# facebookresearch/iSDF

Measured on AMD Instinct MI355X. Metric: train-steps/sec: device-synchronised Trainer.step() on 27k-point ray batches, timed as metrics.start_timing / end_timing bracket it (SURVEY 8d); whole job.  SDF L1 vs GT: sdf_l1_vs_gt, higher is better.
Workload: dtype f16 MFMA operands (compensated forward: hi+lo operands past the cat layer), f32 accumulate; second-order sweeps and dW operands fp16; 1 GPU; replicaCAD.json defaults: 5 keyframes x 200 rays x 27 samples = 27000 points per rank-step, 680x1200 synthetic room depth, 6x256 Softplus MLP + 255-wide icosahedron PE (460033 params), eik+normal loss, bounds=ray, AdamW; stream=680x1200, scaling_mode=weak: every rank draws the full 5 x 200 rays, parallelism=single GPU

## Files before the change

### include/isdf_hip.h

```cpp
#ifndef ISDF_HIP_H
#define ISDF_HIP_H

#include <stddef.h>
#include <stdint.h>

#ifdef __cplusplus
extern "C" {
#endif

#define ISDF_ABI_VERSION 7

enum {
  ISDF_OK = 0,
  ISDF_EINVAL = -1,
  ISDF_EUNSUPPORTED = -2,
  ISDF_EWORKSPACE = -3,
  ISDF_EHIP = -4,
  ISDF_ECOLLECTIVE = -5
};

typedef struct isdf_net_cfg {
  int32_t hidden;
  int32_t blocks;
  int32_t n_freqs;
  int32_t has_transform;
  float scale_input;
  float scale_output;
  float bounds_T[12];
  int32_t fwd_operand;
  int32_t bwd_operand;
  int32_t spill_operand;
} isdf_net_cfg;

int isdf_abi_version(void);
const char* isdf_error_string(int code);

int isdf_check_net(const isdf_net_cfg* net);

int64_t isdf_param_count(const isdf_net_cfg* net);
int64_t isdf_shadow_bytes(const isdf_net_cfg* net);
int64_t isdf_workspace_bytes(const isdf_net_cfg* net, int64_t max_points, int32_t train);
int64_t isdf_reduce_floats(const isdf_net_cfg* net, int32_t n_frames);
int64_t isdf_reduce_split_floats(const isdf_net_cfg* net);

int isdf_pack_weights(const isdf_net_cfg* net, const float* params, void* shadow, void* stream);

typedef struct isdf_sample_args {
  const float* depth_batch;
  const float* normal_batch;
  const float* T_WC_batch;
  const int32_t* frame_idx;
  const int32_t* normal_idx;
  int32_t n_frames;
  int32_t n_rays;
  int32_t H, W;
  float fx, fy, cx, cy;
  int32_t n_strat, n_surf;
  float min_depth;
  float dist_behind_surf;
  int32_t rng_mode;
  const int64_t* draw_h;
  const int64_t* draw_w;
  const float* draw_u;
  const float* draw_n;
  uint64_t seed, offset;
  int32_t n_inline;
  int32_t frame_idx_inline[8];
  int32_t normal_idx_inline[8];
  int32_t reserved_inline;
} isdf_sample_args;
#define ISDF_MAX_INLINE_FRAMES 8

typedef struct isdf_sample_out {
  int32_t* n_valid;
  int64_t* indices_b;
  int64_t* indices_h;
  int64_t* indices_w;
  float* depth_sample;
  float* dirs_C_sample;
  float* norm_sample;
  float* T_WC_sample;
  float* dirs_W_sample;
  float* z_vals;
  float* pc;
} isdf_sample_out;

int64_t isdf_sample_scan_bytes(int64_t max_rays);
int isdf_sample_rays(const isdf_sample_args* a, const isdf_sample_out* o, void* scan_ws,
                     int64_t scan_ws_bytes, void* stream);

int isdf_sdf_eval(const isdf_net_cfg* net, const float* params, const void* shadow,
                  const float* pts, int64_t n_points, const float* noise,
                  float* sdf, float* sdf_grad, void* workspace, int64_t workspace_bytes,
                  void* stream);

typedef struct isdf_loss_cfg {
  int32_t bounds_method;
  int32_t loss_type;
  float trunc_weight, trunc_distance, eik_weight, eik_apply_dist, grad_weight;
  int32_t orien_loss;
} isdf_loss_cfg;

typedef struct isdf_step_args {
  const int32_t* n_valid;
  int32_t max_rays;
  int32_t S;
  int32_t n_frames, H, W;
  const float* pc;
  const float* z_vals;
  const float* depth_sample;
  const float* dirs_C_sample;
  const float* dirs_W_sample;
  const float* norm_sample;
  const int64_t* indices_b;
  const int64_t* indices_h;
  const int64_t* indices_w;
  const float* noise;
  float noise_std;
  uint32_t reserved0;
  uint64_t noise_seed;
  uint64_t noise_offset;
  const float* pc_bounds;
  const float* pc_grad_vec;
  int32_t extra_floats;
  int32_t extra_slot;
  float extra_value;
  int32_t reserved1;
} isdf_step_args;

typedef struct isdf_step_out {
  float* reduce_buf;
  float* sdf;
  float* sdf_grad;
  float* tot_loss_mat;
  void** prof_events;
  float* host_mailbox;
  void* split_event;
} isdf_step_out;

enum { ISDF_LS_SDF = 0, ISDF_LS_GRAD = 1, ISDF_LS_EIK = 2, ISDF_LS_TOTAL = 3, ISDF_LS_COUNT = 4 };

int isdf_train_step(const isdf_net_cfg* net, const isdf_loss_cfg* loss, const float* params,
                    const void* shadow, const isdf_step_args* a, const isdf_step_out* o,
                    void* workspace, int64_t workspace_bytes, void* stream);

typedef struct isdf_optim_args {
  float* params;
  float* exp_avg;
  float* exp_avg_sq;
  void* shadow;
  float lr, beta1, beta2, eps, weight_decay;
  float grad_scale;
  int32_t step;
  int32_t reserved;
  float* loss_approx;
  float* frame_avg;
  const int32_t* frame_avg_index;
  int32_t frame_avg_inline_n;
  int32_t frame_avg_index_inline[8];
  int32_t reserved_inline;
} isdf_optim_args;

int isdf_train_step_adamw(const isdf_net_cfg* net, const isdf_loss_cfg* loss, const isdf_step_args* a,
                          const isdf_step_out* o, const isdf_optim_args* opt, void* workspace,
                          int64_t workspace_bytes, void* stream);

int isdf_train_step_finish(const isdf_net_cfg* net, const isdf_optim_args* opt, const float* reduce_buf,
                           int32_t n_frames, int32_t extra_floats, float* host_mailbox, void* stream);

typedef int (*isdf_nccl_allreduce_fn)(const void* sendbuf, void* recvbuf, size_t count, int datatype, int op,
                                      void* comm, void* stream);
int isdf_allreduce_sum_f32(isdf_nccl_allreduce_fn nccl_all_reduce, void* comm, float* buf, int64_t count, void* stream);

int isdf_bounds_pc(const int32_t* n_valid, int32_t max_rays, int32_t S, const float* pc,
                   const float* z_vals, const float* depth_sample, const float* surf_pts,
                   int64_t n_surf, float* bounds, float* grad_vec, void* stream);

int isdf_frame_avg(const float* reduce_buf, int64_t n_params, int32_t n_frames,
                   float* loss_approx, float* frame_avg_loss, const int32_t* frame_avg_index,
                   void* stream);

int isdf_estimate_normals(const float* depth, int32_t H, int32_t W, float fx, float fy, float cx,
                          float cy, float* normals, void* stream);

int isdf_render_depth(const int32_t* n_valid, int64_t n_rays_host, int64_t max_rays, int32_t S,
                      const float* z_vals, const float* sdf, const float* depth_sample,
                      float kf_dist_th, float* view_depth, int32_t* below_count, void* stream);

int isdf_adamw(const isdf_net_cfg* net, float* params, float* exp_avg, float* exp_avg_sq,
               const float* grad_sum, const float* count_ptr, float grad_scale,
               float lr, float beta1, float beta2, float eps, float weight_decay,
               int32_t step, void* shadow, void* stream);

#ifdef __cplusplus
}
#endif
#endif
```

### isdf_amd/_ffi.py

```python
import ctypes as C
import os

HERE = os.path.dirname(os.path.abspath(__file__))
LIB_PATH = os.environ.get("ISDF_HIP_LIB") or os.path.join(HERE, "libisdf_hip.so")

ABI_VERSION = 7

SYMBOLS = [
    "isdf_abi_version", "isdf_error_string", "isdf_check_net", "isdf_param_count", "isdf_shadow_bytes",
    "isdf_workspace_bytes", "isdf_reduce_floats", "isdf_reduce_split_floats", "isdf_sample_scan_bytes", "isdf_pack_weights",
    "isdf_sample_rays",
    "isdf_sdf_eval", "isdf_train_step", "isdf_train_step_adamw", "isdf_train_step_finish", "isdf_bounds_pc",
    "isdf_frame_avg", "isdf_adamw", "isdf_estimate_normals", "isdf_render_depth", "isdf_allreduce_sum_f32",
]

LS_SDF, LS_GRAD, LS_EIK, LS_TOTAL, LS_COUNT = 0, 1, 2, 3, 4


class NetCfg(C.Structure):
    _fields_ = [("hidden", C.c_int32), ("blocks", C.c_int32), ("n_freqs", C.c_int32),
                ("has_transform", C.c_int32), ("scale_input", C.c_float),
                ("scale_output", C.c_float), ("bounds_T", C.c_float * 12),
                ("fwd_operand", C.c_int32), ("bwd_operand", C.c_int32), ("spill_operand", C.c_int32)]


class SampleArgs(C.Structure):
    _fields_ = [("depth_batch", C.c_void_p), ("normal_batch", C.c_void_p),
                ("T_WC_batch", C.c_void_p), ("frame_idx", C.c_void_p), ("normal_idx", C.c_void_p),
                ("n_frames", C.c_int32), ("n_rays", C.c_int32), ("H", C.c_int32), ("W", C.c_int32),
                ("fx", C.c_float), ("fy", C.c_float), ("cx", C.c_float), ("cy", C.c_float),
                ("n_strat", C.c_int32), ("n_surf", C.c_int32), ("min_depth", C.c_float),
                ("dist_behind_surf", C.c_float), ("rng_mode", C.c_int32),
                ("draw_h", C.c_void_p), ("draw_w", C.c_void_p), ("draw_u", C.c_void_p),
                ("draw_n", C.c_void_p), ("seed", C.c_uint64), ("offset", C.c_uint64),
                ("n_inline", C.c_int32), ("frame_idx_inline", C.c_int32 * 8), ("normal_idx_inline", C.c_int32 * 8),
                ("reserved_inline", C.c_int32)]


class SampleOut(C.Structure):
    _fields_ = [(n, C.c_void_p) for n in
                ["n_valid", "indices_b", "indices_h", "indices_w", "depth_sample", "dirs_C_sample",
                 "norm_sample", "T_WC_sample", "dirs_W_sample", "z_vals", "pc"]]


class LossCfg(C.Structure):
    _fields_ = [("bounds_method", C.c_int32), ("loss_type", C.c_int32),
                ("trunc_weight", C.c_float), ("trunc_distance", C.c_float),
                ("eik_weight", C.c_float), ("eik_apply_dist", C.c_float),
                ("grad_weight", C.c_float), ("orien_loss", C.c_int32)]


class StepArgs(C.Structure):
    _fields_ = [("n_valid", C.c_void_p), ("max_rays", C.c_int32), ("S", C.c_int32),
                ("n_frames", C.c_int32), ("H", C.c_int32), ("W", C.c_int32),
                ("pc", C.c_void_p), ("z_vals", C.c_void_p), ("depth_sample", C.c_void_p),
                ("dirs_C_sample", C.c_void_p), ("dirs_W_sample", C.c_void_p),
                ("norm_sample", C.c_void_p), ("indices_b", C.c_void_p), ("indices_h", C.c_void_p),
                ("indices_w", C.c_void_p), ("noise", C.c_void_p), ("noise_std", C.c_float),
                ("reserved0", C.c_uint32), ("noise_seed", C.c_uint64), ("noise_offset", C.c_uint64),
                ("pc_bounds", C.c_void_p),
                ("pc_grad_vec", C.c_void_p), ("extra_floats", C.c_int32), ("extra_slot", C.c_int32),
                ("extra_value", C.c_float), ("reserved1", C.c_int32)]


class StepOut(C.Structure):
    _fields_ = [("reduce_buf", C.c_void_p), ("sdf", C.c_void_p), ("sdf_grad", C.c_void_p),
                ("tot_loss_mat", C.c_void_p), ("prof_events", C.POINTER(C.c_void_p)), ("host_mailbox", C.c_void_p),
                ("split_event", C.c_void_p)]


class OptimArgs(C.Structure):
    _fields_ = [("params", C.c_void_p), ("exp_avg", C.c_void_p), ("exp_avg_sq", C.c_void_p), ("shadow", C.c_void_p),
                ("lr", C.c_float), ("beta1", C.c_float), ("beta2", C.c_float), ("eps", C.c_float),
                ("weight_decay", C.c_float), ("grad_scale", C.c_float), ("step", C.c_int32), ("reserved", C.c_int32),
                ("loss_approx", C.c_void_p), ("frame_avg", C.c_void_p), ("frame_avg_index", C.c_void_p),
                ("frame_avg_inline_n", C.c_int32), ("frame_avg_index_inline", C.c_int32 * 8), ("reserved_inline", C.c_int32)]
MAX_INLINE_FRAMES = 8



class IsdfError(RuntimeError):
    pass


_lib = None


def lib():
    global _lib
    if _lib is not None:
        return _lib
    if not os.path.exists(LIB_PATH):
        raise IsdfError("%s not found: run `python -m isdf_amd.build` (or __graft_entry__.build())"
                        % LIB_PATH)
    import torch
    L = C.CDLL(LIB_PATH)
    P, i32, i64, f32, vp = C.POINTER, C.c_int32, C.c_int64, C.c_float, C.c_void_p
    L.isdf_abi_version.restype = C.c_int
    L.isdf_error_string.restype = C.c_char_p
    L.isdf_error_string.argtypes = [C.c_int]
    L.isdf_check_net.restype = C.c_int
    L.isdf_check_net.argtypes = [P(NetCfg)]
    for n in ("isdf_param_count", "isdf_shadow_bytes", "isdf_reduce_split_floats"):
        getattr(L, n).restype = i64
        getattr(L, n).argtypes = [P(NetCfg)]
    L.isdf_workspace_bytes.restype = i64
    L.isdf_workspace_bytes.argtypes = [P(NetCfg), i64, i32]
    L.isdf_reduce_floats.restype = i64
    L.isdf_reduce_floats.argtypes = [P(NetCfg), i32]
    L.isdf_pack_weights.argtypes = [P(NetCfg), vp, vp, vp]
    L.isdf_sample_scan_bytes.restype = i64
    L.isdf_sample_scan_bytes.argtypes = [i64]
    L.isdf_sample_rays.argtypes = [P(SampleArgs), P(SampleOut), vp, i64, vp]
    L.isdf_sdf_eval.argtypes = [P(NetCfg), vp, vp, vp, i64, vp, vp, vp, vp, i64, vp]
    L.isdf_train_step.argtypes = [P(NetCfg), P(LossCfg), vp, vp, P(StepArgs), P(StepOut), vp, i64, vp]
    L.isdf_train_step_adamw.argtypes = [P(NetCfg), P(LossCfg), P(StepArgs), P(StepOut), P(OptimArgs), vp, i64, vp]
    L.isdf_train_step_finish.argtypes = [P(NetCfg), P(OptimArgs), vp, i32, i32, vp, vp]
    L.isdf_allreduce_sum_f32.argtypes = [vp, vp, vp, C.c_int64, vp]
    L.isdf_bounds_pc.argtypes = [vp, i32, i32, vp, vp, vp, vp, i64, vp, vp, vp]
    L.isdf_frame_avg.argtypes = [vp, i64, i32, vp, vp, vp, vp]
    L.isdf_adamw.argtypes = [P(NetCfg), vp, vp, vp, vp, vp, f32, f32, f32, f32, f32, f32, i32, vp, vp]
    L.isdf_estimate_normals.argtypes = [vp, i32, i32, f32, f32, f32, f32, vp, vp]
    L.isdf_render_depth.argtypes = [vp, i64, i64, i32, vp, vp, vp, f32, vp, vp, vp]
    for n in SYMBOLS[SYMBOLS.index("isdf_pack_weights"):]:
        getattr(L, n).restype = C.c_int
    if L.isdf_abi_version() != ABI_VERSION:
        raise IsdfError("libisdf_hip.so ABI %d != binding ABI %d" % (L.isdf_abi_version(), ABI_VERSION))
    _lib = L
    return L


def check(rc, what):
    if rc != 0:
        raise IsdfError("%s failed: %s (%d)" % (what, lib().isdf_error_string(int(rc)).decode(), rc))


def ptr(t):
    return None if t is None else C.c_void_p(t.data_ptr())
```

### isdf_amd/csrc/capi.hip

```cpp
#include <cstdio>
#include "isdf_common.h"
#include "chain_params.h"

using namespace isdf;

namespace isdf {
int launch_chain(const ChainParams& p, int mode, int64_t nTiles, hipStream_t st);
int launch_dw(const DwParams& p, hipStream_t st);
int launch_sample_rays(const isdf_sample_args& a, const isdf_sample_out& o, void* scan_ws, hipStream_t st);
int64_t sample_scan_bytes(int64_t max_rays);
int launch_adamw(float* p, float* m, float* v, const float* g, const float* cnt, float gs, float lr, float b1,
                 float b2, float eps, float wd, int step, int64_t n, hipStream_t st);
int launch_pack(const NetLayout& L, const float* params, uint16_t* shadow, hipStream_t st);
int launch_adamw_pack(const NetLayout& L, float* params, float* m, float* v, uint16_t* shadow, const float* grad,
                      const float* count_ptr, float grad_scale, float lr, float b1, float b2, float eps, float wd,
                      int step, hipStream_t st, int n_frames = 0, const float* bl = nullptr, const float* bc = nullptr,
                      float* la = nullptr, float* fa = nullptr, const int32_t* fa_index = nullptr,
                      const float* loss_sums = nullptr, const float* extra = nullptr, int n_extra = 0, float* mailbox = nullptr,
                      int fa_inline_n = 0, const int32_t* fa_inline = nullptr);
int launch_step_tail(int phase, const NetLayout& L, const float* dwPart, const float* vecPart, int vecStride, float* grad,
                     float* params, float* m, float* v, uint16_t* shadow, float grad_scale, float lr, float b1, float b2,
                     float eps, float wd, int step, const float* wg_loss, int64_t maxTiles, const int32_t* n_valid, int S,
                     const float* tot_ws, const int64_t* ib, const int64_t* ih, const int64_t* iw, int F, int H, int W,
                     float* loss_sums, float* bl, float* bc, float* la_out, float* fa_out, const int32_t* fa_index,
                     hipStream_t st, float* mailbox, float* extra, int n_extra, int extra_slot, float extra_value, int part = 0,
                     int fa_inline_n = 0, const int32_t* fa_inline = nullptr);
int launch_frame_avg(const float* bl, const float* bc, int F, float* la, float* fa, const int32_t* fa_index,
                     hipStream_t st);
int launch_bounds_pc(const int32_t* n_valid, int max_rays, int S, const float* pc, const float* z, const float* depth,
                     const float* surf, int64_t n_surf, float* bounds, float* gv, hipStream_t st);
int launch_normals(const float* depth, int H, int W, float fx, float fy, float cx, float cy, float* normals,
                   hipStream_t st);
int launch_render_depth(const int32_t* n_valid, int64_t n_host, int64_t max_rays, int S, const float* z,
                        const float* sdf, const float* depth_sample, float th, float* view, int32_t* below,
                        hipStream_t st);
}

namespace isdf { thread_local int g_isdf_last_hip_error = 0; }

extern "C" {

int isdf_abi_version(void) { return ISDF_ABI_VERSION; }

static thread_local int g_isdf_last_collective_error = 0;

const char* isdf_error_string(int code) {
  switch (code) {
    case ISDF_OK: return "ok";
    case ISDF_EINVAL: return "invalid argument";
    case ISDF_EUNSUPPORTED: return "unsupported configuration (the tile kernels take hidden_feature_size <= 512 (zero-padded to 256 / 512), n_freqs = n_embed_funcs+1 in 1..12, any hidden_layers_block up to 7; bounds_method ray|pc)";
    case ISDF_EWORKSPACE: return "workspace too small";
    case ISDF_EHIP: {
      static thread_local char buf[160];
      snprintf(buf, sizeof(buf), "HIP runtime error: %s", g_isdf_last_hip_error ? hipGetErrorString((hipError_t)g_isdf_last_hip_error) : "(no launch status recorded)");
      return buf;
    }
    case ISDF_ECOLLECTIVE: {
      static thread_local char buf[96];
      snprintf(buf, sizeof(buf), "the collective library refused the all-reduce (ncclResult_t %d)", g_isdf_last_collective_error);
      return buf;
    }
  }
  return "unknown error";
}

int isdf_check_net(const isdf_net_cfg* net) {
  NetLayout l; int rc = make_layout(net, &l);
  if (rc) return rc;
  return layout_supported(l) ? ISDF_OK : ISDF_EUNSUPPORTED;
}

int64_t isdf_param_count(const isdf_net_cfg* net) {
  NetLayout l; int rc = make_layout(net, &l);
  return rc ? rc : l.n_params;
}

int64_t isdf_shadow_bytes(const isdf_net_cfg* net) {
  NetLayout l; int rc = make_layout(net, &l);
  return rc ? rc : l.shadowElems * 2;
}

int64_t isdf_workspace_bytes(const isdf_net_cfg* net, int64_t max_points, int32_t train) {
  NetLayout l; int rc = make_layout(net, &l);
  if (rc) return rc;
  if (max_points < 0) return ISDF_EINVAL;
  WorkspaceLayout w; make_workspace(l, max_points, max_points, train != 0, &w);
  return w.totalBytes;
}

int64_t isdf_reduce_floats(const isdf_net_cfg* net, int32_t n_frames) {
  NetLayout l; int rc = make_layout(net, &l);
  if (rc) return rc;
  return l.n_params + 8 + 2 * (int64_t)n_frames * 64;
}

int64_t isdf_reduce_split_floats(const isdf_net_cfg* net) {
  NetLayout l; int rc = make_layout(net, &l);
  if (rc) return rc;
  return l.offW[l.cat];
}

int isdf_pack_weights(const isdf_net_cfg* net, const float* params, void* shadow, void* stream) {
  isdf_clear_stale_hip_error();
  NetLayout l; int rc = make_layout(net, &l);
  if (rc) return rc;
  if (!params || !shadow) return ISDF_EINVAL;
  return launch_pack(l, params, (uint16_t*)shadow, (hipStream_t)stream);
}

int64_t isdf_sample_scan_bytes(int64_t max_rays) { return max_rays < 1 ? ISDF_EINVAL : sample_scan_bytes(max_rays); }

int isdf_sample_rays(const isdf_sample_args* a, const isdf_sample_out* o, void* scan_ws, int64_t scan_ws_bytes,
                     void* stream) {
  isdf_clear_stale_hip_error();
  if (!a || !o || !a->depth_batch || !a->T_WC_batch || !o->n_valid || !o->indices_b ||
      !o->indices_h || !o->indices_w || !o->depth_sample || !o->dirs_C_sample || !o->dirs_W_sample || !o->z_vals ||
      !o->pc)
    return ISDF_EINVAL;
  if (a->n_inline != 0 && (a->n_inline != a->n_frames || a->n_inline > ISDF_MAX_INLINE_FRAMES)) return ISDF_EINVAL;
  for (int f = 0; f < a->n_inline; ++f)
    if (a->frame_idx_inline[f] < 0 || (a->normal_batch && a->normal_idx_inline[f] < 0)) return ISDF_EINVAL;
  if (a->n_inline == 0 && (!a->frame_idx || (a->normal_batch && !a->normal_idx))) return ISDF_EINVAL;
  if (a->n_frames < 1 || a->n_rays < 1 || a->H < 1 || a->W < 1 || a->n_strat < 1 || a->n_surf < 0) return ISDF_EINVAL;
  if ((int64_t)a->n_frames * a->n_rays > 0x7fffffff / 64) return ISDF_EINVAL;
  if (a->rng_mode == 0 && (!a->draw_h || !a->draw_w || !a->draw_u || (a->n_surf > 1 && !a->draw_n))) return ISDF_EINVAL;
  if (!scan_ws || scan_ws_bytes < sample_scan_bytes((int64_t)a->n_frames * a->n_rays)) return ISDF_EWORKSPACE;
  return launch_sample_rays(*a, *o, scan_ws, (hipStream_t)stream);
}

int isdf_sdf_eval(const isdf_net_cfg* net, const float* params, const void* shadow, const float* pts,
                  int64_t n_points, const float* noise, float* sdf, float* sdf_grad, void* workspace,
                  int64_t workspace_bytes, void* stream) {
  isdf_clear_stale_hip_error();
  NetLayout l; int rc = make_layout(net, &l);
  if (rc) return rc;
  if (!layout_supported(l)) return ISDF_EUNSUPPORTED;
  if (!params || !shadow || !pts || !sdf || n_points < 0) return ISDF_EINVAL;
  if (n_points == 0) return ISDF_OK;
  ChainParams p = {};
  p.lay = l; p.params = params; p.shadow = (const uint16_t*)shadow; p.pts = pts; p.noise = noise;
  p.n_points_host = n_points; p.S = 1; p.sdf = sdf; p.sdf_grad = sdf_grad;
  const int mode = sdf_grad ? 1 : 0;
  WorkspaceLayout w; make_workspace(l, n_points, 0, false, &w);
  if (mode == 1) {
    if (!workspace || workspace_bytes < w.totalBytes) return ISDF_EWORKSPACE;
    p.spill = (uint16_t*)((char*)workspace + w.offSpill); p.sp = w.sp;
  }
  chain_debug_from_env(p.dbg, workspace && workspace_bytes >= 4096 ? (char*)workspace + workspace_bytes - 4096 : nullptr);
  return launch_chain(p, mode, w.nTiles, (hipStream_t)stream);
}

static int train_step_impl(const isdf_net_cfg* net, const isdf_loss_cfg* loss, const float* params, const void* shadow,
                           const isdf_step_args* a, const isdf_step_out* o, void* workspace, int64_t workspace_bytes,
                           void* stream, const isdf_optim_args* opt) {
  isdf_clear_stale_hip_error();
  NetLayout l; int rc = make_layout(net, &l);
  if (rc) return rc;
  if (!layout_supported(l)) return ISDF_EUNSUPPORTED;
  if (!loss || !params || !shadow || !a || !o || !workspace || !o->reduce_buf) return ISDF_EINVAL;
  if (!a->pc || !a->z_vals || !a->depth_sample || !a->dirs_C_sample || !a->dirs_W_sample || !a->indices_b ||
      !a->indices_h || !a->indices_w || !a->n_valid)
    return ISDF_EINVAL;
  if (a->max_rays < 1 || a->S < 1 || a->n_frames < 1 || a->H < 8 || a->W < 8) return ISDF_EINVAL;
  if (a->H % 8 != 0 || a->W % 8 != 0 || a->H >= 65536 || a->W >= 65536) return ISDF_EINVAL;
  if (loss->bounds_method != 0 && loss->bounds_method != 1) return ISDF_EUNSUPPORTED;
  if (loss->bounds_method == 1 && (!a->pc_bounds || !a->pc_grad_vec)) return ISDF_EINVAL;
  if (loss->loss_type != 0 && loss->loss_type != 1) return ISDF_EINVAL;
  if (loss->grad_weight != 0.f && !a->norm_sample) return ISDF_EINVAL;
  const int64_t maxPts = (int64_t)a->max_rays * a->S;
  if (maxPts > 0x7fffffff) return ISDF_EINVAL;
  if (a->extra_floats < 0 || a->extra_floats > 1016 || (a->extra_floats > 0 && (a->extra_slot < 0 || a->extra_slot >= a->extra_floats)))
    return ISDF_EINVAL;
  WorkspaceLayout w; make_workspace(l, maxPts, a->max_rays, true, &w);
  if (workspace_bytes < w.totalBytes) return ISDF_EWORKSPACE;
  hipStream_t st = (hipStream_t)stream;
  char* ws = (char*)workspace;
  float* wgLoss = (float*)(ws + w.offWgLoss);
  float* dwPart = (float*)(ws + w.offDwPart);
  float* vecPart = (float*)(ws + w.offVecPart);
  float* totLoss = (float*)(ws + w.offTotLoss);

  ChainParams p = {};
  p.lay = l; p.loss = *loss; p.params = params; p.shadow = (const uint16_t*)shadow;
  p.pts = a->pc; p.noise = a->noise; p.n_valid = a->n_valid; p.S = a->S;
  p.noise_std = a->noise_std; p.noise_seed = a->noise_seed; p.noise_off = a->noise_offset;
  p.z_vals = a->z_vals; p.depth = a->depth_sample; p.dirsC = a->dirs_C_sample; p.dirsW = a->dirs_W_sample;
  p.normals = a->norm_sample; p.pc_bounds = a->pc_bounds; p.pc_grad_vec = a->pc_grad_vec;
  p.sdf = o->sdf; p.sdf_grad = o->sdf_grad; p.tot_loss_mat = o->tot_loss_mat;
  p.tot_ws = totLoss; p.wg_loss = wgLoss; p.vec_part = vecPart; p.vecStride = w.vecStride;
  p.spill = (uint16_t*)(ws + w.offSpill); p.sp = w.sp;
  p.pe_aux = (float*)(ws + w.offPeAux);
  chain_debug_from_env(p.dbg, ws + w.totalBytes - 4096);
  hipEvent_t* ev = (hipEvent_t*)o->prof_events;
  if (ev && hipEventRecord(ev[0], st) != hipSuccess) return ISDF_EHIP;
  rc = launch_chain(p, 2, w.nTiles, st);
  if (rc) return rc;
  if (ev && hipEventRecord(ev[1], st) != hipSuccess) return ISDF_EHIP;

  DwParams d = {};
  d.lay = l; d.sp = w.sp; d.spill = p.spill; d.pe_aux = p.pe_aux; d.n_valid = a->n_valid; d.S = a->S; d.dwPart = dwPart;
  rc = launch_dw(d, st);
  if (rc) return rc;
  if (ev && hipEventRecord(ev[2], st) != hipSuccess) return ISDF_EHIP;
  float* lossSums = o->reduce_buf + l.n_params;
  float* blockLoss = lossSums + 8;
  float* blockCnt = blockLoss + (int64_t)a->n_frames * 64;
  float* extra = blockCnt + (int64_t)a->n_frames * 64;
  if (opt) {
    rc = launch_step_tail(0, l, dwPart, vecPart, w.vecStride, o->reduce_buf, opt->params, opt->exp_avg, opt->exp_avg_sq,
                          (uint16_t*)opt->shadow, opt->grad_scale, opt->lr, opt->beta1, opt->beta2, opt->eps,
                          opt->weight_decay, opt->step, wgLoss, w.nTiles, a->n_valid, a->S, totLoss, a->indices_b,
                          a->indices_h, a->indices_w, a->n_frames, a->H, a->W, lossSums, blockLoss, blockCnt,
                          opt->loss_approx, opt->frame_avg, opt->frame_avg_index, st, o->host_mailbox, extra, a->extra_floats,
                          a->extra_slot, a->extra_value, 0, opt->frame_avg_inline_n, opt->frame_avg_index_inline);
    if (rc) return rc;
    if (ev && hipEventRecord(ev[3], st) != hipSuccess) return ISDF_EHIP;
    return ISDF_OK;
  }
  const int parts = o->split_event ? 2 : 1;
  for (int part = 1; part <= parts; ++part) {
    rc = launch_step_tail(1, l, dwPart, vecPart, w.vecStride, o->reduce_buf, nullptr, nullptr, nullptr, nullptr, 1.f, 0.f,
                          0.f, 0.f, 0.f, 0.f, 1, wgLoss, w.nTiles, a->n_valid, a->S, totLoss, a->indices_b, a->indices_h,
                          a->indices_w, a->n_frames, a->H, a->W, lossSums, blockLoss, blockCnt, nullptr, nullptr, nullptr,
                          st, o->host_mailbox, extra, a->extra_floats, a->extra_slot, a->extra_value, parts == 1 ? 0 : part);
    if (rc) return rc;
    if (parts == 2 && part == 1 && hipEventRecord((hipEvent_t)o->split_event, st) != hipSuccess) return ISDF_EHIP;
  }
  if (ev && hipEventRecord(ev[3], st) != hipSuccess) return ISDF_EHIP;
  return ISDF_OK;
}

int isdf_train_step(const isdf_net_cfg* net, const isdf_loss_cfg* loss, const float* params,
                    const void* shadow, const isdf_step_args* a, const isdf_step_out* o,
                    void* workspace, int64_t workspace_bytes, void* stream) {
  return train_step_impl(net, loss, params, shadow, a, o, workspace, workspace_bytes, stream, nullptr);
}

int isdf_train_step_adamw(const isdf_net_cfg* net, const isdf_loss_cfg* loss, const isdf_step_args* a,
                          const isdf_step_out* o, const isdf_optim_args* opt, void* workspace,
                          int64_t workspace_bytes, void* stream) {
  if (!a || !opt || !opt->params || !opt->exp_avg || !opt->exp_avg_sq || !opt->shadow || opt->step < 1) return ISDF_EINVAL;
  if ((opt->loss_approx == nullptr) != (opt->frame_avg == nullptr)) return ISDF_EINVAL;
  if (opt->frame_avg_inline_n != 0 && (opt->frame_avg_inline_n != a->n_frames || opt->frame_avg_inline_n > ISDF_MAX_INLINE_FRAMES))
    return ISDF_EINVAL;
  for (int f = 0; f < opt->frame_avg_inline_n; ++f)
    if (opt->frame_avg_index_inline[f] < 0) return ISDF_EINVAL;
  if (o && o->split_event) return ISDF_EINVAL;
  return train_step_impl(net, loss, opt->params, opt->shadow, a, o, workspace, workspace_bytes, stream, opt);
}

int isdf_train_step_finish(const isdf_net_cfg* net, const isdf_optim_args* opt, const float* reduce_buf, int32_t n_frames,
                           int32_t extra_floats, float* host_mailbox, void* stream) {
  isdf_clear_stale_hip_error();
  NetLayout l; int rc = make_layout(net, &l);
  if (rc) return rc;
  if (!layout_supported(l)) return ISDF_EUNSUPPORTED;
  if (!opt || !opt->params || !opt->exp_avg || !opt->exp_avg_sq || !opt->shadow || opt->step < 1 || !reduce_buf) return ISDF_EINVAL;
  if ((opt->loss_approx == nullptr) != (opt->frame_avg == nullptr)) return ISDF_EINVAL;
  if (opt->loss_approx && n_frames < 1) return ISDF_EINVAL;
  if (opt->frame_avg_inline_n != 0 && (opt->frame_avg_inline_n != n_frames || opt->frame_avg_inline_n > ISDF_MAX_INLINE_FRAMES))
    return ISDF_EINVAL;
  for (int f = 0; f < opt->frame_avg_inline_n; ++f)
    if (opt->frame_avg_index_inline[f] < 0) return ISDF_EINVAL;
  if (extra_floats < 0 || extra_floats > 1016 || n_frames < 0) return ISDF_EINVAL;
  if (extra_floats > 0 && !host_mailbox) return ISDF_EINVAL;
  const float* lossSums = reduce_buf + l.n_params;
  const float* bl = lossSums + 8;
  const int F = opt->loss_approx ? n_frames : 0;
  return launch_adamw_pack(l, opt->params, opt->exp_avg, opt->exp_avg_sq, (uint16_t*)opt->shadow, reduce_buf,
                           lossSums + ISDF_LS_COUNT, opt->grad_scale, opt->lr, opt->beta1, opt->beta2, opt->eps,
                           opt->weight_decay, opt->step, (hipStream_t)stream, F, bl, bl + (int64_t)n_frames * 64,
                           opt->loss_approx, opt->frame_avg, opt->frame_avg_index, lossSums, bl + (int64_t)n_frames * 128,
                           extra_floats, host_mailbox, opt->frame_avg_inline_n, opt->frame_avg_index_inline);
}

int isdf_allreduce_sum_f32(isdf_nccl_allreduce_fn nccl_all_reduce, void* comm, float* buf, int64_t count, void* stream) {
  if (!nccl_all_reduce || !comm || !buf || count < 1) return ISDF_EINVAL;
  constexpr int kNcclFloat32 = 7, kNcclSum = 0;
  const int rc = nccl_all_reduce(buf, buf, (size_t)count, kNcclFloat32, kNcclSum, comm, stream);
  if (rc != 0) { g_isdf_last_collective_error = rc; return ISDF_ECOLLECTIVE; }
  return ISDF_OK;
}

int isdf_bounds_pc(const int32_t* n_valid, int32_t max_rays, int32_t S, const float* pc, const float* z_vals,
                   const float* depth_sample, const float* surf_pts, int64_t n_surf, float* bounds, float* grad_vec,
                   void* stream) {
  isdf_clear_stale_hip_error();
  if (!n_valid || !pc || !z_vals || !depth_sample || !bounds || !grad_vec || max_rays < 1 || S < 1) return ISDF_EINVAL;
  if (surf_pts && n_surf < 1) return ISDF_EINVAL;
  return launch_bounds_pc(n_valid, max_rays, S, pc, z_vals, depth_sample, surf_pts, n_surf, bounds, grad_vec,
                          (hipStream_t)stream);
}

int isdf_frame_avg(const float* reduce_buf, int64_t n_params, int32_t n_frames, float* loss_approx,
                   float* frame_avg_loss, const int32_t* frame_avg_index, void* stream) {
  isdf_clear_stale_hip_error();
  if (!reduce_buf || !loss_approx || !frame_avg_loss || n_frames < 1 || n_params < 0) return ISDF_EINVAL;
  const float* bl = reduce_buf + n_params + 8;
  return launch_frame_avg(bl, bl + (int64_t)n_frames * 64, n_frames, loss_approx, frame_avg_loss, frame_avg_index,
                          (hipStream_t)stream);
}

int isdf_estimate_normals(const float* depth, int32_t H, int32_t W, float fx, float fy, float cx, float cy,
                          float* normals, void* stream) {
  isdf_clear_stale_hip_error();
  if (!depth || !normals || H < 1 || W < 1 || fx == 0.f || fy == 0.f) return ISDF_EINVAL;
  return launch_normals(depth, H, W, fx, fy, cx, cy, normals, (hipStream_t)stream);
}

int isdf_render_depth(const int32_t* n_valid, int64_t n_rays_host, int64_t max_rays, int32_t S, const float* z_vals,
                      const float* sdf, const float* depth_sample, float kf_dist_th, float* view_depth,
                      int32_t* below_count, void* stream) {
  isdf_clear_stale_hip_error();
  if (!z_vals || !sdf || !view_depth || S < 1 || max_rays < 1) return ISDF_EINVAL;
  if (!n_valid && (n_rays_host < 0 || n_rays_host > max_rays)) return ISDF_EINVAL;
  return launch_render_depth(n_valid, n_rays_host, max_rays, S, z_vals, sdf, depth_sample, kf_dist_th, view_depth,
                             below_count, (hipStream_t)stream);
}

int isdf_adamw(const isdf_net_cfg* net, float* params, float* exp_avg, float* exp_avg_sq, const float* grad_sum,
               const float* count_ptr, float grad_scale, float lr, float beta1, float beta2, float eps,
               float weight_decay, int32_t step, void* shadow, void* stream) {
  isdf_clear_stale_hip_error();
  NetLayout l; int rc = make_layout(net, &l);
  if (rc) return rc;
  if (!params || !exp_avg || !exp_avg_sq || !grad_sum || step < 1) return ISDF_EINVAL;
  if (shadow && layout_supported(l))
    return launch_adamw_pack(l, params, exp_avg, exp_avg_sq, (uint16_t*)shadow, grad_sum, count_ptr, grad_scale, lr,
                             beta1, beta2, eps, weight_decay, step, (hipStream_t)stream);
  rc = launch_adamw(params, exp_avg, exp_avg_sq, grad_sum, count_ptr, grad_scale, lr, beta1, beta2, eps, weight_decay,
                    step, l.n_params, (hipStream_t)stream);
  if (rc || !shadow) return rc;
  return launch_pack(l, params, (uint16_t*)shadow, (hipStream_t)stream);
}

}
```

### isdf_amd/csrc/isdf_common.h

```cpp
#pragma once
#include <hip/hip_runtime.h>
#include <stdint.h>
#include "../../include/isdf_hip.h"

namespace isdf {

constexpr int MAXL = 16;
constexpr int N_DIRS = 21;
constexpr int TILE_PTS = 64;
constexpr int DW_PTS = 64;
constexpr int CHAIN_NW = 8;
constexpr int CHAIN_CHUNK_FRAGS = 8;
constexpr int DW_SPLIT_REG = 32, DW_SPLIT_PE = 48, DW_SPLIT_MAX = 48;
typedef float slab_t;

typedef __attribute__((ext_vector_type(8))) _Float16 f16x8;
typedef __attribute__((ext_vector_type(4))) _Float16 f16x4;
typedef __attribute__((ext_vector_type(8))) __bf16 bf16x8;
typedef __attribute__((ext_vector_type(4))) __bf16 bf16x4;
typedef __attribute__((ext_vector_type(16))) float f32x16;
typedef __attribute__((ext_vector_type(4))) float f32x4;
typedef __attribute__((ext_vector_type(2))) float f32x2;

struct NetLayout {
  int HD, EP, E, B, L, cat, n_freqs;
  int H;
  int fwd_f16;
  int fwd_x2;
  int fwd_x2_all;
  int bwd_f16;
  int sp8;
  int has_transform;
  float scale_input, scale_output;
  float T[12];
  int64_t n_params;
  int32_t offW[MAXL], offB[MAXL], K[MAXL];
  int32_t offWout, offBout;
  int64_t fwdMat[MAXL];
  int64_t bwdMat[MAXL];
  int64_t bwdG;
  int64_t fwdSetElems, bwdSetElems;
  int64_t setFwdA, setFwdB, setBwdA, setBwdB;
  int64_t setFwdLo;
  int64_t shadowElems;
};

constexpr float kSpillPScale = 1.f / 1024.f;
struct SpillLayout {
  int64_t tensorElems;
  int64_t tileStride;
  int64_t A[MAXL + 1];
  int64_t P[MAXL];
  int64_t GB[MAXL];
  int64_t ZB[MAXL];
  int64_t totalElems;
};

struct WorkspaceLayout {
  int64_t nTiles;
  SpillLayout sp;
  int64_t offSpill;
  int64_t offWgLoss;
  int64_t offDwPart;
  int64_t offVecPart;
  int64_t offTotLoss;
  int64_t offPeAux;
  int32_t vecStride;
  int64_t totalBytes;
};

#if defined(__HIPCC__)
extern thread_local int g_isdf_last_hip_error;
inline void isdf_clear_stale_hip_error() { (void)hipGetLastError(); }
inline int isdf_launch_status() {
  const hipError_t e = hipGetLastError();
  if (e == hipSuccess) return ISDF_OK;
  g_isdf_last_hip_error = (int)e;
  return ISDF_EHIP;
}
#endif

inline int round_up(int x, int m) { return (x + m - 1) / m * m; }

__host__ __device__ inline int spill_gb_shift(int n_freqs) { return n_freqs > 6 ? n_freqs - 7 : -1; }

inline int make_layout(const isdf_net_cfg* c, NetLayout* l) {
  if (!c || !l) return ISDF_EINVAL;
  if (c->blocks < 1 || 2 * c->blocks + 2 > MAXL || c->n_freqs < 1 || c->hidden < 1) return ISDF_EINVAL;
  l->H = c->hidden; l->HD = c->hidden <= 256 ? 256 : 512; l->B = c->blocks; l->n_freqs = c->n_freqs;
  if (c->hidden > 512) return ISDF_EUNSUPPORTED;
  l->E = 2 * N_DIRS * c->n_freqs + 3;
  l->EP = round_up(l->E, 256) > l->HD ? round_up(l->E, 256) : l->HD;
  l->L = 2 * c->blocks + 2; l->cat = c->blocks + 1;
  if (c->fwd_operand < 0 || c->fwd_operand > 3) return ISDF_EINVAL;
  l->fwd_f16 = c->fwd_operand ? 1 : 0;
  l->fwd_x2 = c->fwd_operand >= 2 ? 1 : 0;
  l->fwd_x2_all = c->fwd_operand == 3 ? 1 : 0;
  if (c->bwd_operand < 0 || c->bwd_operand > 1 || (c->bwd_operand == 1 && !l->fwd_f16)) return ISDF_EINVAL;
  l->bwd_f16 = c->bwd_operand;
  if (c->spill_operand < 0 || c->spill_operand > 3 || (c->spill_operand >= 2 && !l->bwd_f16)) return ISDF_EINVAL;
  if (c->spill_operand >= 2 && l->HD != 256) return ISDF_EUNSUPPORTED;
  l->sp8 = c->spill_operand == 2 ? 3 : c->spill_operand == 3 ? 1 : (c->spill_operand == 0 && l->bwd_f16 && c->n_freqs <= 6 && l->HD == 256) ? 3 : 0;
  l->has_transform = c->has_transform;
  l->scale_input = c->scale_input; l->scale_output = c->scale_output;
  for (int i = 0; i < 12; ++i) l->T[i] = c->has_transform ? c->bounds_T[i] : (i % 5 == 0 ? 1.f : 0.f);
  int64_t off = 0;
  for (int li = 0; li < l->L; ++li) {
    int K = li == 0 ? l->E : (li == l->cat ? l->H + l->E : l->H);
    l->K[li] = K;
    l->offW[li] = (int32_t)off; off += (int64_t)l->H * K;
    l->offB[li] = (int32_t)off; off += l->H;
  }
  l->offWout = (int32_t)off; off += l->H;
  l->offBout = (int32_t)off; off += 1;
  l->n_params = off;
  int64_t f = 0, b = 0;
  for (int li = 0; li < l->L; ++li) {
    int Kp = li == 0 ? l->EP : (li == l->cat ? l->HD + l->EP : l->HD);
    l->fwdMat[li] = f; f += (int64_t)l->HD * Kp;
    l->bwdMat[li] = b; if (li >= 1) b += (int64_t)l->HD * l->HD;
  }
  l->bwdG = b; b += (int64_t)l->EP * 2 * l->HD;
  l->fwdSetElems = f; l->bwdSetElems = b;
  l->setFwdA = 0; l->setFwdB = f; l->setBwdA = 2 * f; l->setBwdB = 2 * f + b;
  l->setFwdLo = 2 * f + 2 * b;
  l->shadowElems = 2 * f + 2 * b + (l->fwd_x2 ? f : 0);
  return ISDF_OK;
}

inline bool layout_supported(const NetLayout& l) {
  if (l.fwd_x2_all) return l.HD == 256 && l.EP == 256;
  return (l.HD == 256 && (l.EP == 256 || l.EP == 512)) || (l.HD == 512 && l.EP == 512);
}

constexpr int DW_BLK = 256;
struct DwUnit { int li, ob, ib; };
__host__ __device__ inline int dw_kpad(const NetLayout& l, int li) {
  return li == 0 ? l.EP : (li == l.cat ? l.HD + l.EP : l.HD);
}
__host__ __device__ inline int dw_units(const NetLayout& l) {
  int n = 0;
  for (int li = 0; li < l.L; ++li) n += (l.HD / DW_BLK) * (dw_kpad(l, li) / DW_BLK);
  return n;
}
__host__ __device__ inline DwUnit dw_unit(const NetLayout& l, int u) {
  const int nOb = l.HD / DW_BLK;
  for (int li = 0; li < l.L; ++li) {
    const int n = nOb * (dw_kpad(l, li) / DW_BLK);
    if (u < n) return DwUnit{li, u % nOb, u / nOb};
    u -= n;
  }
  return DwUnit{0, 0, 0};
}

__host__ __device__ inline bool dw_unit_from_emb(const NetLayout& l, const DwUnit& du) {
  return du.li == 0 || (du.li == l.cat && du.ib * DW_BLK >= l.HD);
}
__host__ __device__ inline int dw_unit_splits(const NetLayout& l, int u) {
  return dw_unit_from_emb(l, dw_unit(l, u)) ? DW_SPLIT_PE : DW_SPLIT_REG;
}
__host__ __device__ inline int dw_slab_base(const NetLayout& l, int u) {
  int n = 0;
  for (int v = 0; v < u; ++v) n += dw_unit_splits(l, v);
  return n;
}
__host__ __device__ inline int dw_total_slabs(const NetLayout& l) { return dw_slab_base(l, dw_units(l)); }

inline void make_workspace(const NetLayout& l, int64_t maxPts, int64_t maxRays, bool train, WorkspaceLayout* w) {
  w->nTiles = (maxPts + TILE_PTS - 1) / TILE_PTS;
  SpillLayout& s = w->sp;
  s.tensorElems = TILE_PTS * (int64_t)l.HD;
  int64_t o = 0;
  s.A[0] = -1;
  for (int i = 1; i <= l.L; ++i) { s.A[i] = o; o += s.tensorElems; }
  if (train) {
    for (int i = 0; i < l.L; ++i) { s.P[i] = o; o += ((l.sp8 & 2) && i < l.L - 1) ? s.tensorElems / 2 : s.tensorElems; }
    s.GB[0] = -1;
    for (int i = 1; i < l.L; ++i) { s.GB[i] = o; o += (l.sp8 & 1) ? s.tensorElems / 2 : s.tensorElems; }
    for (int i = 0; i < l.L; ++i) { s.ZB[i] = o; o += s.tensorElems; }
  }
  s.tileStride = o;
  s.totalElems = o * w->nTiles;
  o = s.totalElems;
  int64_t b = 0;
  w->offSpill = b; b += o * 2; b = (b + 255) / 256 * 256;
  (void)maxRays;
  w->offWgLoss = b; b += (train ? w->nTiles * 8 : 0) * 4; b = (b + 255) / 256 * 256;
  w->offDwPart = b; b += train ? (int64_t)dw_total_slabs(l) * DW_BLK * DW_BLK * 4 : 0; b = (b + 255) / 256 * 256;
  w->vecStride = round_up(l.L * l.HD + 2 * l.HD + 8, 64);
  w->offVecPart = b; b += train ? w->nTiles * (int64_t)w->vecStride * 4 : 0; b = (b + 255) / 256 * 256;
  w->offTotLoss = b; b += train ? maxPts * 4 : 0; b = (b + 255) / 256 * 256;
  w->offPeAux = b; b += train ? w->nTiles * TILE_PTS * 8 * 4 : 0; b = (b + 255) / 256 * 256;
  w->totalBytes = b + 256 + 4096;
}

#if defined(__HIPCC__)

static __constant__ float kDirs[3][N_DIRS] = {
    {0.8506508f, 0.809017f, 0.5257311f, 1.f, 0.809017f, 0.8506508f, 0.309017f, 0.f, 0.5f, 0.f, -0.5257311f,
     -0.309017f, 0.f, -0.309017f, 0.309017f, 0.5f, 0.5f, 0.f, -0.5f, -0.809017f, -0.809017f},
    {0.f, 0.5f, 0.8506508f, 0.f, 0.5f, 0.f, 0.809017f, 0.5257311f, 0.309017f, 1.f, 0.8506508f, 0.809017f,
     0.5257311f, 0.809017f, 0.809017f, 0.309017f, -0.309017f, 0.f, 0.309017f, 0.5f, 0.5f},
    {0.5257311f, 0.309017f, 0.f, 0.f, -0.309017f, -0.5257311f, -0.5f, -0.8506508f, -0.809017f, 0.f, 0.f,
     -0.5f, 0.8506508f, 0.5f, 0.5f, 0.809017f, 0.809017f, 1.f, 0.809017f, 0.309017f, -0.309017f}};

template <bool F16> struct Op;
template <> struct Op<true> {
  typedef f16x8 v8; typedef f16x4 v4; typedef _Float16 e;
  static __device__ __forceinline__ f32x16 mfma(v8 a, v8 b, f32x16 c) {
    return __builtin_amdgcn_mfma_f32_32x32x16_f16(a, b, c, 0, 0, 0);
  }
  static __device__ __forceinline__ float clampf(float x) { return x; }
};
template <> struct Op<false> {
  typedef bf16x8 v8; typedef bf16x4 v4; typedef __bf16 e;
  static __device__ __forceinline__ f32x16 mfma(v8 a, v8 b, f32x16 c) {
    return __builtin_amdgcn_mfma_f32_32x32x16_bf16(a, b, c, 0, 0, 0);
  }
  static __device__ __forceinline__ float clampf(float x) { return x; }
};

template <bool F16> __device__ __forceinline__ uint2 pack4(float a, float b, float c, float d) {
  typename Op<F16>::v4 v;
  v[0] = (typename Op<F16>::e)Op<F16>::clampf(a); v[1] = (typename Op<F16>::e)Op<F16>::clampf(b);
  v[2] = (typename Op<F16>::e)Op<F16>::clampf(c); v[3] = (typename Op<F16>::e)Op<F16>::clampf(d);
  return __builtin_bit_cast(uint2, v);
}
__device__ __forceinline__ float f16_residual(float v) { return v - (float)(_Float16)v; }
__device__ __forceinline__ void unpack4_bf16(uint2 u, float (&o)[4]) {
  o[0] = __uint_as_float(u.x << 16); o[1] = __uint_as_float(u.x & 0xffff0000u);
  o[2] = __uint_as_float(u.y << 16); o[3] = __uint_as_float(u.y & 0xffff0000u);
}

__device__ __forceinline__ uint4 philox4x32_10(uint4 ctr, uint2 key) {
  constexpr uint32_t M0 = 0xD2511F53u, M1 = 0xCD9E8D57u, W0 = 0x9E3779B9u, W1 = 0xBB67AE85u;
#pragma unroll
  for (int r = 0; r < 10; ++r) {
    const uint32_t hi0 = __umulhi(M0, ctr.x), lo0 = M0 * ctr.x;
    const uint32_t hi1 = __umulhi(M1, ctr.z), lo1 = M1 * ctr.z;
    ctr = make_uint4(hi1 ^ ctr.y ^ key.x, lo1, hi0 ^ ctr.w ^ key.y, lo0);
    key.x += W0; key.y += W1;
  }
  return ctr;
}
__device__ __forceinline__ float u01(uint32_t x) { return (x >> 8) * (1.0f / 16777216.0f); }


#endif
}
```

### isdf_amd/csrc/optim.hip

```cpp
#include "isdf_common.h"

namespace isdf {

struct AdamwCoef { float lr, b1, b2, eps, wd, bc1, bc2_sqrt; };
__device__ __forceinline__ float adamw_update(float* __restrict__ p, float* __restrict__ m, float* __restrict__ v,
                                              int64_t i, float gsum, float gs, const AdamwCoef& c) {
#pragma clang fp contract(off)
  const float gi = gsum * gs;
  float pi = p[i] * (1.f - c.lr * c.wd);
  const float m0 = m[i], v0 = v[i];
  const float mi = c.b1 * m0 + (1.f - c.b1) * gi;
  const float vi = c.b2 * v0 + (1.f - c.b2) * gi * gi;
  const float denom = sqrtf(vi) / c.bc2_sqrt + c.eps;
  pi -= (c.lr / c.bc1) * (mi / denom);
  p[i] = pi;
  m[i] = mi; v[i] = vi;
  return pi;
}
__global__ void adamw_kernel(float* __restrict__ p, float* __restrict__ m, float* __restrict__ v,
                             const float* __restrict__ g, const float* __restrict__ count_ptr,
                             float grad_scale, AdamwCoef c, int64_t n) {
  const int64_t i = (int64_t)blockIdx.x * blockDim.x + threadIdx.x;
  if (i >= n) return;
  float gs = grad_scale;
  if (count_ptr) { if (*count_ptr == 0.f) return; gs /= *count_ptr; }
  adamw_update(p, m, v, i, g[i], gs, c);
}

__device__ __forceinline__ float fwd_src(const NetLayout& L, const float* P, int li, int row, int k) {
  const int HD = L.HD, H = L.H;
  if (row >= H) return 0.f;
  if (li == 0) return k < L.E ? P[L.offW[0] + (int64_t)row * L.K[0] + k] : 0.f;
  if (li == L.cat) {
    if (k < HD) return k < H ? P[L.offW[li] + (int64_t)row * L.K[li] + k] : 0.f;
    const int e = k - HD;
    return e < L.E ? P[L.offW[li] + (int64_t)row * L.K[li] + H + e] : 0.f;
  }
  return k < H ? P[L.offW[li] + (int64_t)row * L.K[li] + k] : 0.f;
}
__device__ __forceinline__ float bwd_src(const NetLayout& L, const float* P, int li, int row, int k) {
  return (row < L.H && k < L.H) ? P[L.offW[li] + (int64_t)k * L.K[li] + row] : 0.f;
}
__device__ __forceinline__ float g_src(const NetLayout& L, const float* P, int row, int k) {
  if (row >= L.E) return 0.f;
  if (k < L.HD) return k < L.H ? P[L.offW[0] + (int64_t)k * L.K[0] + row] : 0.f;
  return k - L.HD < L.H ? P[L.offW[L.cat] + (int64_t)(k - L.HD) * L.K[L.cat] + L.H + row] : 0.f;
}

__global__ void pack_kernel(NetLayout L, const float* __restrict__ P, uint16_t* __restrict__ shadow) {
  const int64_t gid = (int64_t)blockIdx.x * blockDim.x + threadIdx.x;
  const int64_t perFwd = L.fwdSetElems / 8, perBwd = L.bwdSetElems / 8;
  if (gid >= perFwd + perBwd) return;
  const bool isFwd = gid < perFwd;
  const int64_t e0 = (isFwd ? gid : gid - perFwd) * 8;
  float v[8];
  if (isFwd) {
    int li = 0;
    for (int k = 1; k < L.L; ++k) if (e0 >= L.fwdMat[k]) li = k;
    const int Kp = li == 0 ? L.EP : (li == L.cat ? L.HD + L.EP : L.HD);
    int64_t r = (e0 - L.fwdMat[li]) / 8;
    const int lane = (int)(r & 63); r >>= 6;
    const int ks = (int)(r % (Kp / 16)); const int rb = (int)(r / (Kp / 16));
    const int row = rb * 32 + (lane & 31), k0 = ks * 16 + 8 * (lane >> 5);
#pragma unroll
    for (int t = 0; t < 8; ++t) v[t] = fwd_src(L, P, li, row, k0 + t);
  } else {
    const bool isG = e0 >= L.bwdG;
    int li = 1;
    if (!isG) for (int k = 2; k < L.L; ++k) if (e0 >= L.bwdMat[k]) li = k;
    const int Kp = isG ? 2 * L.HD : L.HD;
    int64_t r = (e0 - (isG ? L.bwdG : L.bwdMat[li])) / 8;
    const int lane = (int)(r & 63); r >>= 6;
    const int ks = (int)(r % (Kp / 16)); const int rb = (int)(r / (Kp / 16));
    const int row = rb * 32 + (lane & 31), k0 = ks * 16 + 8 * (lane >> 5);
#pragma unroll
    for (int t = 0; t < 8; ++t) v[t] = isG ? g_src(L, P, row, k0 + t) : bwd_src(L, P, li, row, k0 + t);
  }
  const uint2 a16 = pack4<true>(v[0], v[1], v[2], v[3]), b16 = pack4<true>(v[4], v[5], v[6], v[7]);
  const uint2 abf = pack4<false>(v[0], v[1], v[2], v[3]), bbf = pack4<false>(v[4], v[5], v[6], v[7]);
  const uint4 hA = L.fwd_f16 ? make_uint4(a16.x, a16.y, b16.x, b16.y) : make_uint4(abf.x, abf.y, bbf.x, bbf.y);
  const uint4 hB = make_uint4(abf.x, abf.y, bbf.x, bbf.y);
  *(uint4*)(shadow + (isFwd ? L.setFwdA : L.setBwdA) + e0) = hA;
  if (!L.bwd_f16) *(uint4*)(shadow + (isFwd ? L.setFwdB : L.setBwdB) + e0) = hB;
  if (L.fwd_x2 && isFwd && (L.fwd_x2_all || e0 >= L.fwdMat[L.cat])) {
    float r[8];
#pragma unroll
    for (int t = 0; t < 8; ++t) r[t] = f16_residual(v[t]);
    const uint2 al = pack4<true>(r[0], r[1], r[2], r[3]), bl = pack4<true>(r[4], r[5], r[6], r[7]);
    *(uint4*)(shadow + L.setFwdLo + e0) = make_uint4(al.x, al.y, bl.x, bl.y);
  }
}

constexpr int FIN_CAP = 12288;
struct FinalizeArgs {
  const float* wg_loss; int64_t maxTiles; const int32_t* n_valid; int S; const float* tot_ws;
  const int64_t *ib, *ih, *iw; int n_frames, H, W;
  float *loss_sums, *block_loss, *block_cnt;
  float *la_out, *fa_out; const int32_t* fa_index;
  int fa_inline_n; int32_t fa_inline[8];
  float* mailbox; float* extra; int n_extra, extra_slot; float extra_value;
};
struct FinalizeLds { float sh[16][8]; unsigned long long binS[64]; float binC[64]; int range[2]; int cnt[16][2]; uint32_t keys[FIN_CAP]; };

__device__ __forceinline__ void finalize_block(int block, const FinalizeArgs& a, FinalizeLds& lds) {
  const float* __restrict__ wg_loss = a.wg_loss; const int64_t maxTiles = a.maxTiles; const int S = a.S;
  const float* __restrict__ tot_ws = a.tot_ws;
  const int64_t* __restrict__ ib = a.ib; const int64_t* __restrict__ ih = a.ih; const int64_t* __restrict__ iw = a.iw;
  const int H = a.H, W = a.W;
  float* __restrict__ loss_sums = a.loss_sums; float* __restrict__ block_loss = a.block_loss;
  float* __restrict__ block_cnt = a.block_cnt;
  auto& sh = lds.sh; auto& binS = lds.binS; auto& binC = lds.binC; auto& range = lds.range; auto& keys = lds.keys;
  const int tid = threadIdx.x, lane = tid & 63, wv = tid >> 6;
  const int64_t R = *a.n_valid;
  const int64_t P = R * S;
  if (block == 0) {
    const int64_t nTiles = (P + TILE_PTS - 1) / TILE_PTS;
    float acc[5] = {0.f, 0.f, 0.f, 0.f, 0.f};
    for (int64_t t = tid; t < nTiles && t < maxTiles; t += 1024)
#pragma unroll
      for (int k = 0; k < 5; ++k) acc[k] += wg_loss[t * 8 + k];
#pragma unroll
    for (int k = 0; k < 5; ++k) {
      float v = acc[k];
#pragma unroll
      for (int m = 32; m >= 1; m >>= 1) v += __shfl_xor(v, m, 64);
      if (lane == 0) sh[wv][k] = v;
    }
    __syncthreads();
    if (tid < 8) {
      float v = 0.f;
      if (tid < 5) for (int k = 0; k < 16; ++k) v += sh[k][tid];
      loss_sums[tid] = v;
      if (a.mailbox) a.mailbox[tid] = v;
    }
    if (tid < a.n_extra) a.extra[tid] = tid == a.extra_slot ? a.extra_value : 0.f;
    return;
  }
  const int f = block - 1;
  {
    int c0 = 0, c1 = 0;
    for (int64_t r = tid; r < R; r += 1024) { const int64_t b = ib[r]; c0 += b < f; c1 += b <= f; }
#pragma unroll
    for (int m = 32; m >= 1; m >>= 1) { c0 += __shfl_xor(c0, m, 64); c1 += __shfl_xor(c1, m, 64); }
    if (lane == 0) { lds.cnt[wv][0] = c0; lds.cnt[wv][1] = c1; }
  }
  if (tid < 64) { binS[tid] = 0ull; binC[tid] = 0.f; }
  __syncthreads();
  if (tid < 2) {
    int c = 0;
    for (int k = 0; k < 16; ++k) c += lds.cnt[k][tid];
    range[tid] = c;
  }
  __syncthreads();
  const int lo = range[0], n = range[1] - range[0];
  const bool staged = n <= FIN_CAP;
  if (staged) for (int r = tid; r < n; r += 1024) keys[r] = ((uint32_t)ih[lo + r] << 16) | (uint32_t)iw[lo + r];
  __syncthreads();
  const int hb = H / 8, wb = W / 8;
  for (int r = tid; r < n; r += 1024) {
    const uint32_t h = (uint32_t)ih[lo + r], w = (uint32_t)iw[lo + r];
    const uint32_t key = (h << 16) | w;
    bool dup = false;
    if (staged) { for (int q = r + 1; q < n; ++q) dup |= keys[q] == key; }
    else { for (int q = r + 1; q < n; ++q) dup |= ((((uint32_t)ih[lo + q]) << 16) | (uint32_t)iw[lo + q]) == key; }
    if (dup) continue;
    float s = 0.f;
    const float* tp = tot_ws + (int64_t)(lo + r) * S;
    for (int k = 0; k < S; ++k) s += tp[k];
    const int bin = (int)((h / hb) * 8 + (w / wb));
    atomicAdd(&binS[bin], (unsigned long long)(long long)llrint((double)s * 4294967296.0));
    atomicAdd(&binC[bin], 1.f);
  }
  __syncthreads();
  if (tid < 64) {
    const float bs = (float)((double)(long long)binS[tid] * (1.0 / 4294967296.0));
    block_loss[f * 64 + tid] = bs; block_cnt[f * 64 + tid] = binC[tid];
    if (a.la_out) {
      float c = binC[tid];
      c = c == 0.f ? 1.f : c;
      float v = bs / c;
      a.la_out[f * 64 + tid] = v;
#pragma unroll
      for (int m = 32; m >= 1; m >>= 1) v += __shfl_xor(v, m, 64);
      if (tid == 0) a.fa_out[a.fa_inline_n ? a.fa_inline[f] : (a.fa_index ? a.fa_index[f] : f)] = v / 64.f;
    }
  }
}

struct TailParams {
  NetLayout lay;
  const float* dwPart; const float* vecPart; int32_t vecStride;
  float* grad;
  float *params, *m, *v; uint16_t* shadow;
  AdamwCoef c; float grad_scale;
  const float* count_ptr;
  FinalizeArgs fin;
  int nW, nV;
  int wBlock0;
};

__device__ __forceinline__ void shadow_put(const NetLayout& L, uint16_t* sh, bool fwdSet, int64_t elem, float val,
                                           bool withResidual = false) {
  const uint32_t h = pack4<true>(val, 0.f, 0.f, 0.f).x & 0xffffu, b = pack4<false>(val, 0.f, 0.f, 0.f).x & 0xffffu;
  sh[(fwdSet ? L.setFwdA : L.setBwdA) + elem] = (uint16_t)(L.fwd_f16 ? h : b);
  if (!L.bwd_f16) sh[(fwdSet ? L.setFwdB : L.setBwdB) + elem] = (uint16_t)b;
  if (withResidual) sh[L.setFwdLo + elem] = (uint16_t)(pack4<true>(f16_residual(val), 0.f, 0.f, 0.f).x & 0xffffu);
}
__device__ __forceinline__ int64_t packed_elem(int row, int k, int Kp) {
  return ((((int64_t)(row >> 5) * (Kp >> 4) + (k >> 4)) * 64 + (row & 31) + 32 * ((k & 15) >> 3)) << 3) + (k & 7);
}

__device__ __forceinline__ void frame_avg_block(int f, int t, const float* __restrict__ block_loss,
                                                const float* __restrict__ block_cnt, float* __restrict__ loss_approx,
                                                float* __restrict__ frame_avg, const int32_t* __restrict__ fa_index,
                                                int dst_inline = -1) {
  if (t >= 64) return;
  float c = block_cnt[f * 64 + t];
  c = c == 0.f ? 1.f : c;
  float v = block_loss[f * 64 + t] / c;
  loss_approx[f * 64 + t] = v;
#pragma unroll
  for (int m = 32; m >= 1; m >>= 1) v += __shfl_xor(v, m, 64);
  if (t == 0) frame_avg[dst_inline >= 0 ? dst_inline : (fa_index ? fa_index[f] : f)] = v / 64.f;
}

template <int PHASE>
__global__ __launch_bounds__(1024) void step_tail_kernel(const TailParams p) {
  __shared__ FinalizeLds lds;
  const NetLayout& L = p.lay;
  const int HD = L.HD;
  const int b = blockIdx.x;
  if (b >= p.nW + p.nV) {
    if (PHASE != 2) finalize_block(b - p.nW - p.nV, p.fin, lds);
    else if (b - p.nW - p.nV < p.fin.n_frames)
      frame_avg_block(b - p.nW - p.nV, threadIdx.x, p.fin.block_loss, p.fin.block_cnt, p.fin.la_out, p.fin.fa_out, p.fin.fa_index,
                      p.fin.fa_inline_n ? p.fin.fa_inline[b - p.nW - p.nV] : -1);
    else if ((int)threadIdx.x < 8 + p.fin.n_extra)
      p.fin.mailbox[threadIdx.x] = threadIdx.x < 8 ? p.fin.loss_sums[threadIdx.x] : p.fin.extra[threadIdx.x - 8];
    return;
  }
  const int64_t P = PHASE == 2 ? 0 : (int64_t)(*p.fin.n_valid) * p.fin.S;
  float gs = p.grad_scale;
  if (PHASE == 0) gs /= (float)P;
  if (PHASE == 2 && p.count_ptr) gs /= *p.count_ptr;
  const bool emptyBatch = (PHASE == 0 && P == 0) || (PHASE == 2 && p.count_ptr && *p.count_ptr == 0.f);
  if (b < p.nW) {
    const int64_t idx = (int64_t)(b + p.wBlock0) * 1024 + threadIdx.x;
    constexpr int64_t perUnit = (int64_t)DW_BLK * DW_BLK;
    const int unit = (int)(idx / perUnit);
    if (unit >= dw_units(L)) return;
    const DwUnit du = dw_unit(L, unit);
    const int rem = (int)(idx - unit * perUnit);
    const int o = du.ob * DW_BLK + rem / DW_BLK;
    const int ip = du.ib * DW_BLK + rem % DW_BLK;
    const int li = du.li;
    if (o >= L.H) return;
    if (li == 0 && ip >= L.E) return;
    if (li == L.cat && ip >= HD && ip - HD >= L.E) return;
    if ((li != 0 && ip < HD && ip >= L.H)) return;
    const int col = (li == L.cat && ip >= HD) ? L.H + (ip - HD) : ip;
    const int64_t pi = L.offW[li] + (int64_t)o * L.K[li] + col;
    float s = 0.f;
    if (PHASE == 2) s = p.grad[pi];
    else {
      const slab_t* src = (const slab_t*)p.dwPart + (int64_t)dw_slab_base(L, unit) * perUnit + rem;
#pragma unroll
      for (int k = 0; k < DW_SPLIT_REG; ++k) s += __builtin_nontemporal_load(src + (int64_t)k * perUnit);
      if (dw_unit_from_emb(L, du)) {
#pragma unroll
        for (int k = DW_SPLIT_REG; k < DW_SPLIT_PE; ++k) s += __builtin_nontemporal_load(src + (int64_t)k * perUnit);
      }
      p.grad[pi] = s;
      if (PHASE == 1) return;
    }
    if (emptyBatch) return;
    const float w = adamw_update(p.params, p.m, p.v, pi, s, gs, p.c);
    const int KpF = li == 0 ? L.EP : (li == L.cat ? HD + L.EP : HD);
    shadow_put(L, p.shadow, true, L.fwdMat[li] + packed_elem(o, ip, KpF), w, L.fwd_x2 && (L.fwd_x2_all || li >= L.cat));
    if (li >= 1 && ip < HD) shadow_put(L, p.shadow, false, L.bwdMat[li] + packed_elem(ip, o, HD), w);
    if (li == 0) shadow_put(L, p.shadow, false, L.bwdG + packed_elem(ip, o, 2 * HD), w);
    else if (li == L.cat && ip >= HD) shadow_put(L, p.shadow, false, L.bwdG + packed_elem(ip - HD, HD + o, 2 * HD), w);
    return;
  }
  float (*sh)[64] = (float (*)[64])lds.keys;
  const int pi = threadIdx.x & 63, g = threadIdx.x >> 6;
  const int v = (b - p.nW) * 64 + pi;
  const int nVec = L.L * HD + HD + 1;
  const int nTiles = (int)((P + TILE_PTS - 1) / TILE_PTS);
  int slotA = 0, slotB = -1, dst = -1;
  if (v < L.L * HD) { slotA = v; if (v % HD < L.H) dst = L.offB[v / HD] + v % HD; }
  else if (v < L.L * HD + HD) { slotA = v; slotB = v + HD; if (v - L.L * HD < L.H) dst = L.offWout + (v - L.L * HD); }
  else if (v < nVec) { slotA = L.L * HD + 2 * HD; dst = L.offBout; }
  if (PHASE == 2) {
    if (g == 0 && dst >= 0 && !emptyBatch) adamw_update(p.params, p.m, p.v, dst, p.grad[dst], gs, p.c);
    return;
  }
  float s = 0.f, s2 = 0.f;
  if (dst >= 0) {
    int t = g;
    for (; t + 112 < nTiles; t += 128) {
      const float* r0 = p.vecPart + (int64_t)t * p.vecStride;
      float a[8], bb[8];
#pragma unroll
      for (int q = 0; q < 8; ++q) a[q] = r0[(int64_t)(16 * q) * p.vecStride + slotA];
      if (slotB >= 0) {
#pragma unroll
        for (int q = 0; q < 8; ++q) bb[q] = r0[(int64_t)(16 * q) * p.vecStride + slotB];
        s2 += ((bb[0] + bb[1]) + (bb[2] + bb[3])) + ((bb[4] + bb[5]) + (bb[6] + bb[7]));
      }
      s += ((a[0] + a[1]) + (a[2] + a[3])) + ((a[4] + a[5]) + (a[6] + a[7]));
    }
    for (; t + 48 < nTiles; t += 64) {
      const float* r0 = p.vecPart + (int64_t)t * p.vecStride;
      const float a0 = r0[slotA], a1 = r0[(int64_t)16 * p.vecStride + slotA],
                  a2 = r0[(int64_t)32 * p.vecStride + slotA], a3 = r0[(int64_t)48 * p.vecStride + slotA];
      s += (a0 + a1) + (a2 + a3);
      if (slotB >= 0) {
        const float b0 = r0[slotB], b1 = r0[(int64_t)16 * p.vecStride + slotB],
                    b2 = r0[(int64_t)32 * p.vecStride + slotB], b3 = r0[(int64_t)48 * p.vecStride + slotB];
        s2 += (b0 + b1) + (b2 + b3);
      }
    }
    for (; t < nTiles; t += 16) {
      const float* row = p.vecPart + (int64_t)t * p.vecStride;
      s += row[slotA];
      if (slotB >= 0) s2 += row[slotB];
    }
    s += s2;
  }
  sh[g][pi] = s;
  __syncthreads();
  if (g == 0 && dst >= 0) {
    float t = 0.f;
#pragma unroll
    for (int k = 0; k < 16; ++k) t += sh[k][pi];
    p.grad[dst] = t;
    if (PHASE == 0 && !emptyBatch) adamw_update(p.params, p.m, p.v, dst, t, gs, p.c);
  }
}

__global__ void frame_avg_kernel(const float* __restrict__ block_loss, const float* __restrict__ block_cnt,
                                 int n_frames, float* __restrict__ loss_approx, float* __restrict__ frame_avg,
                                 const int32_t* __restrict__ fa_index) {
  frame_avg_block(blockIdx.x, threadIdx.x, block_loss, block_cnt, loss_approx, frame_avg, fa_index);
}

__global__ __launch_bounds__(256) void bounds_pc_kernel(const int32_t* __restrict__ n_valid, int S,
                                                        const float* __restrict__ pc, const float* __restrict__ z_vals,
                                                        const float* __restrict__ depth, const float* __restrict__ surf,
                                                        int64_t n_surf, float* __restrict__ bounds,
                                                        float* __restrict__ grad_vec) {
  __shared__ float sx[256], sy[256], sz[256];
  const int64_t Rl = *n_valid, P = Rl * S;
  const int64_t R = surf ? n_surf : Rl;
  const int64_t sstride = surf ? 3 : (int64_t)S * 3;
  const float* sp = surf ? surf : pc;
  const int64_t n = (int64_t)blockIdx.x * 256 + threadIdx.x;
  if ((int64_t)blockIdx.x * 256 >= P) return;
  float px = 0.f, py = 0.f, pz = 0.f;
  if (n < P) { px = pc[n * 3]; py = pc[n * 3 + 1]; pz = pc[n * 3 + 2]; }
  float best = INFINITY; int64_t bi = 0;
  for (int64_t r0 = 0; r0 < R; r0 += 256) {
    const int64_t r = r0 + threadIdx.x;
    __syncthreads();
    if (r < R) { sx[threadIdx.x] = sp[r * sstride]; sy[threadIdx.x] = sp[r * sstride + 1]; sz[threadIdx.x] = sp[r * sstride + 2]; }
    __syncthreads();
    const int cnt = (int)((R - r0) < 256 ? (R - r0) : 256);
    for (int k = 0; k < cnt; ++k) {
      const float dx = px - sx[k], dy = py - sy[k], dz = pz - sz[k];
      const float d2 = __fadd_rn(__fadd_rn(__fmul_rn(dx, dx), __fmul_rn(dy, dy)), __fmul_rn(dz, dz));
      if (d2 < best) { best = d2; bi = r0 + k; }
    }
  }
  if (n >= P) return;
  const int64_t ray = n / S;
  const float dist = sqrtf(best);
  const bool behind = z_vals[n] > depth[ray];
  bounds[n] = behind ? -dist : dist;
  float gx = px - sp[bi * sstride], gy = py - sp[bi * sstride + 1], gz = pz - sp[bi * sstride + 2];
  const float nn = sqrtf(gx * gx + gy * gy + gz * gz);
  gx /= nn; gy /= nn; gz /= nn;
  if (behind) { gx = -gx; gy = -gy; gz = -gz; }
  grad_vec[n * 3] = gx; grad_vec[n * 3 + 1] = gy; grad_vec[n * 3 + 2] = gz;
}

int launch_adamw(float* p, float* m, float* v, const float* g, const float* cnt, float gs, float lr,
                 float b1, float b2, float eps, float wd, int step, int64_t n, hipStream_t st) {
  const AdamwCoef c = {lr, b1, b2, eps, wd, 1.f - powf(b1, (float)step), sqrtf(1.f - powf(b2, (float)step))};
  hipLaunchKernelGGL(adamw_kernel, dim3((unsigned)((n + 255) / 256)), dim3(256), 0, st, p, m, v, g, cnt, gs, c, n);
  return isdf_launch_status();
}
int launch_pack(const NetLayout& L, const float* params, uint16_t* shadow, hipStream_t st) {
  const int64_t groups = (L.fwdSetElems + L.bwdSetElems) / 8;
  hipLaunchKernelGGL(pack_kernel, dim3((unsigned)((groups + 255) / 256)), dim3(256), 0, st, L, params, shadow);
  return isdf_launch_status();
}
static FinalizeArgs finalize_args(const float* wg_loss, int64_t maxTiles, const int32_t* n_valid, int S, const float* tot_ws,
                                  const int64_t* ib, const int64_t* ih, const int64_t* iw, int F, int H, int W,
                                  float* loss_sums, float* bl, float* bc) {
  FinalizeArgs a = {};
  a.wg_loss = wg_loss; a.maxTiles = maxTiles; a.n_valid = n_valid; a.S = S; a.tot_ws = tot_ws; a.ib = ib; a.ih = ih; a.iw = iw;
  a.n_frames = F; a.H = H; a.W = W; a.loss_sums = loss_sums; a.block_loss = bl; a.block_cnt = bc;
  return a;
}
int launch_step_tail(int phase, const NetLayout& L, const float* dwPart, const float* vecPart, int vecStride, float* grad,
                     float* params, float* m, float* v, uint16_t* shadow, float grad_scale, float lr, float b1, float b2,
                     float eps, float wd, int step, const float* wg_loss, int64_t maxTiles, const int32_t* n_valid, int S,
                     const float* tot_ws, const int64_t* ib, const int64_t* ih, const int64_t* iw, int F, int H, int W,
                     float* loss_sums, float* bl, float* bc, float* la_out, float* fa_out, const int32_t* fa_index,
                     hipStream_t st, float* mailbox, float* extra, int n_extra, int extra_slot, float extra_value, int part,
                     int fa_inline_n, const int32_t* fa_inline) {
  TailParams p = {};
  p.lay = L; p.dwPart = dwPart; p.vecPart = vecPart; p.vecStride = vecStride; p.grad = grad;
  p.params = params; p.m = m; p.v = v; p.shadow = shadow; p.grad_scale = grad_scale;
  if (phase == 0)
    p.c = AdamwCoef{lr, b1, b2, eps, wd, 1.f - powf(b1, (float)step), sqrtf(1.f - powf(b2, (float)step))};
  p.fin = finalize_args(wg_loss, maxTiles, n_valid, S, tot_ws, ib, ih, iw, F, H, W, loss_sums, bl, bc);
  if (la_out && fa_out) {
    p.fin.la_out = la_out; p.fin.fa_out = fa_out; p.fin.fa_index = fa_index;
    p.fin.fa_inline_n = fa_inline_n;
    for (int k = 0; k < fa_inline_n && k < 8; ++k) p.fin.fa_inline[k] = fa_inline[k];
  }
  p.fin.mailbox = mailbox; p.fin.extra = extra; p.fin.n_extra = n_extra; p.fin.extra_slot = extra_slot; p.fin.extra_value = extra_value;
  const int64_t total = (int64_t)dw_units(L) * DW_BLK * DW_BLK;
  p.nW = (int)((total + 1023) / 1024);
  p.nV = (L.L * L.HD + L.HD + 1 + 63) / 64;
  int tailBlocks = p.nV + 1 + F;
  if (part != 0) {
    if (phase != 1) return ISDF_EINVAL;
    int unitsBelow = 0;
    for (int li = 0; li < L.cat; ++li) unitsBelow += (L.HD / DW_BLK) * (dw_kpad(L, li) / DW_BLK);
    const int split = unitsBelow * (DW_BLK * DW_BLK / 1024);
    if (part == 1) { p.wBlock0 = split; p.nW -= split; }
    else { p.nW = split; p.nV = 0; tailBlocks = 0; }
  }
  const dim3 grid((unsigned)(p.nW + tailBlocks));
  if (grid.x == 0) return ISDF_OK;
  if (phase == 0) hipLaunchKernelGGL(step_tail_kernel<0>, grid, dim3(1024), 0, st, p);
  else hipLaunchKernelGGL(step_tail_kernel<1>, grid, dim3(1024), 0, st, p);
  return isdf_launch_status();
}
int launch_adamw_pack(const NetLayout& L, float* params, float* m, float* v, uint16_t* shadow, const float* grad,
                      const float* count_ptr, float grad_scale, float lr, float b1, float b2, float eps, float wd,
                      int step, hipStream_t st, int n_frames = 0, const float* bl = nullptr, const float* bc = nullptr,
                      float* la = nullptr, float* fa = nullptr, const int32_t* fa_index = nullptr,
                      const float* loss_sums = nullptr, const float* extra = nullptr, int n_extra = 0, float* mailbox = nullptr,
                      int fa_inline_n = 0, const int32_t* fa_inline = nullptr) {
  TailParams p = {};
  p.fin.fa_inline_n = fa_inline_n;
  for (int k = 0; k < fa_inline_n && k < 8; ++k) p.fin.fa_inline[k] = fa_inline[k];
  p.fin.block_loss = const_cast<float*>(bl); p.fin.block_cnt = const_cast<float*>(bc);
  p.fin.la_out = la; p.fin.fa_out = fa; p.fin.fa_index = fa_index; p.fin.n_frames = n_frames;
  p.fin.loss_sums = const_cast<float*>(loss_sums); p.fin.extra = const_cast<float*>(extra); p.fin.n_extra = n_extra;
  p.fin.mailbox = mailbox;
  p.lay = L; p.grad = const_cast<float*>(grad); p.params = params; p.m = m; p.v = v; p.shadow = shadow;
  p.grad_scale = grad_scale; p.count_ptr = count_ptr;
  p.c = AdamwCoef{lr, b1, b2, eps, wd, 1.f - powf(b1, (float)step), sqrtf(1.f - powf(b2, (float)step))};
  const int64_t total = (int64_t)dw_units(L) * DW_BLK * DW_BLK;
  p.nW = (int)((total + 1023) / 1024);
  p.nV = (L.L * L.HD + L.HD + 1 + 63) / 64;
  hipLaunchKernelGGL(step_tail_kernel<2>, dim3((unsigned)(p.nW + p.nV + n_frames + (mailbox ? 1 : 0))), dim3(1024), 0, st, p);
  return isdf_launch_status();
}
int launch_frame_avg(const float* bl, const float* bc, int F, float* la, float* fa, const int32_t* fa_index,
                     hipStream_t st) {
  hipLaunchKernelGGL(frame_avg_kernel, dim3(F), dim3(64), 0, st, bl, bc, F, la, fa, fa_index);
  return isdf_launch_status();
}
int launch_bounds_pc(const int32_t* n_valid, int max_rays, int S, const float* pc, const float* z, const float* depth,
                     const float* surf, int64_t n_surf, float* bounds, float* gv, hipStream_t st) {
  const int64_t maxPts = (int64_t)max_rays * S;
  hipLaunchKernelGGL(bounds_pc_kernel, dim3((unsigned)((maxPts + 255) / 256)), dim3(256), 0, st, n_valid, S, pc, z,
                     depth, surf, n_surf, bounds, gv);
  return isdf_launch_status();
}

}
```

### isdf_amd/csrc/sampler.hip

```cpp
#include "isdf_common.h"

namespace isdf {

constexpr int SMP_NT = 1024;
constexpr int SMP_CHUNK_SMALL = 64;
constexpr int SMP_CHUNK_STREAM = 1024;
constexpr int SMP_SMALL_SLOTS = 4;

__device__ __forceinline__ uint4 ray_random(const isdf_sample_args& a, uint32_t ray, uint32_t slot) {
  return philox4x32_10(make_uint4(ray, slot, (uint32_t)a.offset, (uint32_t)(a.offset >> 32)),
                       make_uint2((uint32_t)a.seed, (uint32_t)(a.seed >> 32)));
}

constexpr unsigned long long ST_AGG = 1ull, ST_INC = 2ull;
__device__ __forceinline__ unsigned long long st_pack(uint32_t epoch, unsigned long long flag, uint32_t v) {
  return ((unsigned long long)(epoch & 0x3fffffffu) << 34) | (flag << 32) | v;
}

__device__ __forceinline__ int pick8(const int32_t (&v)[8], int b) {
  int r = v[0];
#pragma unroll
  for (int k = 1; k < 8; ++k) r = b == k ? v[k] : r;
  return r;
}
__device__ __forceinline__ int window_frame(const isdf_sample_args& a, int b) { return a.n_inline ? pick8(a.frame_idx_inline, b) : a.frame_idx[b]; }
__device__ __forceinline__ int window_normal(const isdf_sample_args& a, int b) { return a.n_inline ? pick8(a.normal_idx_inline, b) : a.normal_idx[b]; }

__device__ __forceinline__ bool ray_valid(const isdf_sample_args& a, int r) {
  const int b = r / a.n_rays;
  int h, wq;
  if (a.rng_mode == 0) { h = (int)a.draw_h[r]; wq = (int)a.draw_w[r]; }
  else { const uint4 u = ray_random(a, (uint32_t)r, 0u); h = (int)(u.x % (uint32_t)a.H); wq = (int)(u.y % (uint32_t)a.W); }
  const int64_t pix = (int64_t)h * a.W + wq;
  const float d = a.depth_batch[(int64_t)window_frame(a, b) * a.H * a.W + pix];
  bool valid = d != 0.f;
  if (a.normal_batch) {
    const float n0 = a.normal_batch[((int64_t)window_normal(a, b) * a.H * a.W + pix) * 3];
    valid = valid && !(n0 != n0);
  }
  return valid;
}

template <int CHUNK>
__global__ __launch_bounds__(SMP_NT) void sample_rays_kernel(const isdf_sample_args a, const isdf_sample_out o,
                                                              uint32_t* __restrict__ ws, int nChunks) {
  constexpr bool SMALL = CHUNK == SMP_CHUNK_SMALL;
  constexpr int NT = SMP_NT, NW = NT / 64, GW = CHUNK / 64;
  __shared__ int sChunk, sBase;
  __shared__ uint32_t sEpoch;
  __shared__ int sPre[NW], sWaveCnt[NW];
  __shared__ float sRay[CHUNK][8];
  __shared__ __attribute__((aligned(16))) float sPc[NW][768];
  const int tid = threadIdx.x, lane = tid & 63, wv = tid >> 6;
  unsigned long long* state = (unsigned long long*)(ws + 4);
  const int total = a.n_frames * a.n_rays;
  const int S = a.n_strat + a.n_surf;
  int c = blockIdx.x;
  uint32_t epoch = 0;
  if (!SMALL) {
    if (tid == 0) {
      sEpoch = __hip_atomic_load(ws + 2, __ATOMIC_RELAXED, __HIP_MEMORY_SCOPE_AGENT) + 1u;
      sChunk = (int)atomicAdd(ws, 1u);
    }
    __syncthreads();
    c = sChunk;
    epoch = sEpoch;
  }

  bool valid = false;
  int b = 0, h = 0, wq = 0, before = 0; float d = 0.f, n0 = 0.f, n1 = 0.f, n2 = 0.f;
  const float* T = a.T_WC_batch;
  float Tm[12];
#pragma unroll
  for (int k = 0; k < 12; ++k) Tm[k] = 0.f;
  if (wv < GW) {
    const int r = c * CHUNK + wv * 64 + lane;
    if (r < total) {
      b = r / a.n_rays;
      if (a.rng_mode == 0) { h = (int)a.draw_h[r]; wq = (int)a.draw_w[r]; }
      else { const uint4 u = ray_random(a, (uint32_t)r, 0u); h = (int)(u.x % (uint32_t)a.H); wq = (int)(u.y % (uint32_t)a.W); }
      const int64_t pix = (int64_t)h * a.W + wq;
      const int fi = window_frame(a, b);
      const float* np = a.normal_batch ? a.normal_batch + ((int64_t)window_normal(a, b) * a.H * a.W + pix) * 3 : nullptr;
      d = a.depth_batch[(int64_t)fi * a.H * a.W + pix];
      if (np) { n0 = np[0]; n1 = np[1]; n2 = np[2]; }
      T += (int64_t)fi * 16;
#pragma unroll
      for (int k = 0; k < 12; ++k) Tm[k] = T[k];
      valid = d != 0.f;
      if (np) valid = valid && !(n0 != n0);
    }
    const unsigned long long m = __ballot(valid);
    before = __popcll(m & ((1ull << lane) - 1ull));
    if (lane == 0) sWaveCnt[wv] = __popcll(m);
  }
  if (SMALL) {
    int n = 0;
#pragma unroll
    for (int k = 0; k < SMP_SMALL_SLOTS; ++k) {
      const int r = tid + k * NT;
      if (r < c * CHUNK) n += ray_valid(a, r) ? 1 : 0;
    }
#pragma unroll
    for (int k = 32; k >= 1; k >>= 1) n += __shfl_xor(n, k, 64);
    if (lane == 0) sPre[wv] = n;
  }
  __syncthreads();

  if (wv == 0) {
    int cnt = lane < GW ? sWaveCnt[lane] : 0;
#pragma unroll
    for (int k = 8; k >= 1; k >>= 1) cnt += __shfl_xor(cnt, k, 64);
    cnt = __shfl(cnt, 0, 64);
    int base = 0;
    if (SMALL) {
      int v = lane < NW ? sPre[lane] : 0;
#pragma unroll
      for (int k = 8; k >= 1; k >>= 1) v += __shfl_xor(v, k, 64);
      base = __shfl(v, 0, 64);
    } else if (c == 0) {
      if (lane == 0) __hip_atomic_store(state, st_pack(epoch, ST_INC, (uint32_t)cnt), __ATOMIC_RELAXED, __HIP_MEMORY_SCOPE_AGENT);
    } else {
      if (lane == 0) __hip_atomic_store(state + c, st_pack(epoch, ST_AGG, (uint32_t)cnt), __ATOMIC_RELAXED, __HIP_MEMORY_SCOPE_AGENT);
      int pos = c - 1;
      while (true) {
        const int idx = pos - lane;
        unsigned long long w = 0ull;
        if (idx >= 0) w = __hip_atomic_load(state + idx, __ATOMIC_RELAXED, __HIP_MEMORY_SCOPE_AGENT);
        const bool ready = idx >= 0 && (uint32_t)(w >> 34) == (epoch & 0x3fffffffu) && ((w >> 32) & 3ull) != 0ull;
        const bool inc = ready && ((w >> 32) & 3ull) == ST_INC;
        const unsigned long long rm = __ballot(ready), im = __ballot(inc), vm = __ballot(idx >= 0);
        const int firstInc = im ? __ffsll((long long)im) - 1 : 63;
        const unsigned long long need = (firstInc == 63 ? ~0ull : ((2ull << firstInc) - 1ull)) & vm;
        if ((rm & need) == need) {
          int v = (need >> lane) & 1ull ? (int)(uint32_t)w : 0;
#pragma unroll
          for (int k = 32; k >= 1; k >>= 1) v += __shfl_xor(v, k, 64);
          base += v;
          if (im) break;
          pos -= 64;
        } else {
          __builtin_amdgcn_s_sleep(2);
        }
      }
      if (lane == 0) __hip_atomic_store(state + c, st_pack(epoch, ST_INC, (uint32_t)(base + cnt)), __ATOMIC_RELAXED, __HIP_MEMORY_SCOPE_AGENT);
    }
    if (lane == 0) sBase = base;
    if (c == nChunks - 1 && lane == 0) *o.n_valid = base + cnt;
  }
  __syncthreads();

  int wbase = 0, cnt_ = 0;
#pragma unroll
  for (int k = 0; k < GW; ++k) { const int n = sWaveCnt[k]; if (k < wv) wbase += n; cnt_ += n; }
  const int base = sBase;
  if (wv < GW && valid) {
    const int jl = wbase + before;
    const int64_t q = (int64_t)base + jl;
    o.indices_b[q] = b; o.indices_h[q] = h; o.indices_w[q] = wq;
    o.depth_sample[q] = d;
    if (o.norm_sample) { o.norm_sample[q * 3] = n0; o.norm_sample[q * 3 + 1] = n1; o.norm_sample[q * 3 + 2] = n2; }
    const float dx = ((float)wq - a.cx) / a.fx, dy = ((float)h - a.cy) / a.fy, dz = 1.f;
    o.dirs_C_sample[q * 3] = dx; o.dirs_C_sample[q * 3 + 1] = dy; o.dirs_C_sample[q * 3 + 2] = dz;
    if (o.T_WC_sample) {
      float4* dst = (float4*)(o.T_WC_sample + q * 16);
      dst[0] = make_float4(Tm[0], Tm[1], Tm[2], Tm[3]); dst[1] = make_float4(Tm[4], Tm[5], Tm[6], Tm[7]);
      dst[2] = make_float4(Tm[8], Tm[9], Tm[10], Tm[11]); dst[3] = make_float4(T[12], T[13], T[14], T[15]);
    }
    float* sr = sRay[jl];
    sr[0] = d;
#pragma unroll
    for (int i = 0; i < 3; ++i) {
      const float s = __fadd_rn(__fadd_rn(__fmul_rn(Tm[i * 4], dx), __fmul_rn(Tm[i * 4 + 1], dy)), __fmul_rn(Tm[i * 4 + 2], dz));
      o.dirs_W_sample[q * 3 + i] = s;
      sr[1 + i] = Tm[i * 4 + 3];
      sr[4 + i] = s;
    }
  }
  __syncthreads();

  const int npts = cnt_ * S;
  struct __attribute__((packed, aligned(4))) f4u { float x, y, z, w; };
  for (int G = wv; G * 256 < npts; G += NW) {
    const bool fullGroup = G * 256 + 256 <= npts;
    uint4 rnd = make_uint4(0u, 0u, 0u, 0u);
    if (a.rng_mode != 0) rnd = ray_random(a, (uint32_t)c, 1u + (uint32_t)(G * 64 + lane));
#pragma unroll
   for (int m = 0; m < 4; ++m) {
    const int p = G * 256 + m * 64 + lane;
    if (p >= npts) continue;
    const uint32_t word = m == 0 ? rnd.x : (m == 1 ? rnd.y : (m == 2 ? rnd.z : rnd.w));
    const int j = p / S, s = p - j * S;
    const int64_t r = (int64_t)base + j;
    const float* sr = sRay[j];
    const float depth = sr[0];
    const float maxd = __fadd_rn(depth, a.dist_behind_surf);
    float z;
    if (s < a.n_surf) {
      if (s == 0) z = depth;
      else {
        float off;
        if (a.rng_mode == 0) off = a.draw_n[r * (a.n_surf - 1) + (s - 1)];
        else {
          const float u1 = ((float)(word >> 16) + 0.5f) * (1.f / 65536.f), u2 = (float)(word & 0xffffu) * (1.f / 65536.f);
          off = 0.1f * sqrtf(-2.f * __logf(u1)) * __cosf(6.2831853f * u2);
        }
        z = fminf(fmaxf(__fadd_rn(depth, off), a.min_depth), maxd);
      }
    } else {
      const int k = s - a.n_surf, nb = a.n_strat;
      float U;
      if (a.rng_mode == 0) U = a.draw_u[r * nb + k];
      else U = u01(word);
      const float step = 1.f / (float)nb;
      const float lin = k < (nb + 1) / 2 ? __fmul_rn(step, (float)k) : __fadd_rn(1.f, -__fmul_rn(step, (float)(nb - k)));
      const float range = __fadd_rn(maxd, -a.min_depth);
      const float lim = __fadd_rn(__fmul_rn(lin, range), a.min_depth);
      const float blen = range / (float)nb;
      z = __fadd_rn(lim, __fmul_rn(U, blen));
    }
    const int64_t n = r * S + s;
    o.z_vals[n] = z;
#pragma unroll
    for (int i = 0; i < 3; ++i) {
      const float v = __fadd_rn(sr[1 + i], __fmul_rn(sr[4 + i], z));
      if (fullGroup) sPc[wv][(m * 64 + lane) * 3 + i] = v;
      else o.pc[n * 3 + i] = v;
    }
   }
    if (fullGroup) {
      __builtin_amdgcn_fence(__ATOMIC_RELEASE, "wavefront");
      __builtin_amdgcn_wave_barrier();
      __builtin_amdgcn_fence(__ATOMIC_ACQUIRE, "wavefront");
      float* dst = o.pc + ((int64_t)base * S + (int64_t)G * 256) * 3;
#pragma unroll
      for (int k = 0; k < 3; ++k) {
        const float4 v = *(const float4*)&sPc[wv][(k * 64 + lane) * 4];
        *(f4u*)(dst + (k * 64 + lane) * 4) = f4u{v.x, v.y, v.z, v.w};
      }
      __builtin_amdgcn_wave_barrier();
    }
  }

  if (SMALL) return;
  __syncthreads();
  if (tid == 0) {
    const uint32_t done = atomicAdd(ws + 1, 1u);
    if ((int)done == nChunks - 1) {
      __hip_atomic_store(ws, 0u, __ATOMIC_RELAXED, __HIP_MEMORY_SCOPE_AGENT);
      __hip_atomic_store(ws + 1, 0u, __ATOMIC_RELAXED, __HIP_MEMORY_SCOPE_AGENT);
      __hip_atomic_store(ws + 2, epoch, __ATOMIC_RELAXED, __HIP_MEMORY_SCOPE_AGENT);
    }
  }
}

constexpr int SMP_SMALL_MAX_RAYS = SMP_NT * SMP_SMALL_SLOTS;

int64_t sample_scan_bytes(int64_t max_rays) { return 16 + 8 * ((max_rays + SMP_CHUNK_STREAM - 1) / SMP_CHUNK_STREAM); }

int launch_sample_rays(const isdf_sample_args& a, const isdf_sample_out& o, void* scan_ws, hipStream_t st) {
  const int total = a.n_frames * a.n_rays;
  if (total <= SMP_SMALL_MAX_RAYS) {
    const int nChunks = (total + SMP_CHUNK_SMALL - 1) / SMP_CHUNK_SMALL;
    hipLaunchKernelGGL(sample_rays_kernel<SMP_CHUNK_SMALL>, dim3((unsigned)nChunks), dim3(SMP_NT), 0, st, a, o, (uint32_t*)scan_ws, nChunks);
  } else {
    const int nChunks = (total + SMP_CHUNK_STREAM - 1) / SMP_CHUNK_STREAM;
    hipLaunchKernelGGL(sample_rays_kernel<SMP_CHUNK_STREAM>, dim3((unsigned)nChunks), dim3(SMP_NT), 0, st, a, o, (uint32_t*)scan_ws, nChunks);
  }
  return isdf_launch_status();
}

}
```

### isdf_amd/engine.py

```python
import ctypes as C
from dataclasses import dataclass, field
from typing import Optional

import numpy as np
import torch

from . import _ffi

N_DIRS = 21
FWD_OPERANDS = ("bf16", "fp16", "fp16x2", "fp16x2_full")


@dataclass
class NetConfig:
    hidden: int = 256
    blocks: int = 2
    n_freqs: int = 6
    scale_input: float = 0.05937489
    scale_output: float = 0.14
    transform: Optional[np.ndarray] = None
    fwd_operand: str = "fp16x2"
    bwd_operand: Optional[str] = None
    spill_operand: Optional[str] = None

    @property
    def emb(self):
        return 2 * N_DIRS * self.n_freqs + 3

    def layer_names(self):
        B = self.blocks
        return (["in_layer.0"] + ["mid1.%d.0" % i for i in range(B)] + ["cat_layer.0"]
                + ["mid2.%d.0" % i for i in range(B)])

    def param_shapes(self):
        H, E, B = self.hidden, self.emb, self.blocks
        fan_in = [E] + [H] * B + [H + E] + [H] * B
        out = []
        for n, k in zip(self.layer_names(), fan_in):
            out += [(n + ".weight", (H, k)), (n + ".bias", (H,))]
        out += [("out_alpha.weight", (1, H)), ("out_alpha.bias", (1,))]
        return out

    def to_c(self):
        c = _ffi.NetCfg()
        c.hidden, c.blocks, c.n_freqs = self.hidden, self.blocks, self.n_freqs
        c.has_transform = 0 if self.transform is None else 1
        c.scale_input, c.scale_output = self.scale_input, self.scale_output
        T = np.eye(4, dtype=np.float32) if self.transform is None else np.asarray(self.transform, np.float32)
        for i in range(12):
            c.bounds_T[i] = float(T[i // 4, i % 4])
        if self.fwd_operand not in FWD_OPERANDS:
            raise ValueError("fwd_operand must be one of %s" % (FWD_OPERANDS,))
        c.fwd_operand = FWD_OPERANDS.index(self.fwd_operand)
        bwd = self.bwd_operand or ("bf16" if self.fwd_operand == "bf16" else "fp16")
        if bwd not in ("bf16", "fp16") or (bwd == "fp16" and self.fwd_operand == "bf16"):
            raise ValueError("bwd_operand must be 'bf16' or 'fp16' (fp16 needs an fp16-family fwd_operand)")
        c.bwd_operand = 1 if bwd == "fp16" else 0
        if self.spill_operand not in (None, "auto", "16bit", "e4m3", "e4m3_gb"):
            raise ValueError("spill_operand must be None / 'auto', '16bit', 'e4m3' or 'e4m3_gb'")
        c.spill_operand = {None: 0, "auto": 0, "16bit": 1, "e4m3": 2, "e4m3_gb": 3}[self.spill_operand]
        return c


@dataclass
class LossConfig:
    bounds_method: str = "ray"
    loss_type: str = "L1"
    trunc_weight: float = 5.38344020
    trunc_distance: float = 0.29365022
    eik_weight: float = 0.268
    eik_apply_dist: float = 0.1
    grad_weight: float = 0.018
    orien_loss: bool = False

    def to_c(self):
        if self.bounds_method not in ("ray", "pc"):
            raise ValueError("bounds_method must be 'ray' or 'pc'")
        if self.loss_type not in ("L1", "L2"):
            raise ValueError("Must be L1 or L2")
        c = _ffi.LossCfg()
        c.bounds_method = 0 if self.bounds_method == "ray" else 1
        c.loss_type = 0 if self.loss_type == "L1" else 1
        c.trunc_weight, c.trunc_distance = self.trunc_weight, self.trunc_distance
        c.eik_weight, c.eik_apply_dist = self.eik_weight, self.eik_apply_dist
        c.grad_weight, c.orien_loss = self.grad_weight, int(self.orien_loss)
        return c


@dataclass
class SampleConfig:
    n_rays: int = 200
    n_strat: int = 19
    n_surf: int = 8
    min_depth: float = 0.07
    dist_behind_surf: float = 0.1
    H: int = 680
    W: int = 1200
    fx: float = 600.0
    fy: float = 600.0
    cx: float = 599.5
    cy: float = 339.5

    @property
    def S(self):
        return self.n_strat + self.n_surf


_PINNED = {}


def _stream(device=None):
    idx = torch.cuda.current_device() if device is None or device.index is None else device.index
    p = _PINNED.get(idx)
    if p is not None:
        return p[1]
    return C.c_void_p(torch.cuda.current_stream(idx).cuda_stream)


_RAW_STREAM = getattr(torch._C, "_cuda_getCurrentRawStream", None)
_STREAM_OBJ = {}


class pinned_stream:

    def __init__(self, device=None):
        if isinstance(device, int):
            self.idx = device
        else:
            self.idx = torch.cuda.current_device() if device is None or torch.device(device).index is None else torch.device(device).index

    def __enter__(self):
        self.prev = _PINNED.get(self.idx)
        c = _STREAM_OBJ.get(self.idx)
        if c is None or _RAW_STREAM is None or _RAW_STREAM(self.idx) != c[2]:
            st = torch.cuda.current_stream(self.idx)
            c = _STREAM_OBJ[self.idx] = (st, C.c_void_p(st.cuda_stream), st.cuda_stream)
        _PINNED[self.idx] = c
        return c[0]

    def __exit__(self, *exc):
        if self.prev is None:
            _PINNED.pop(self.idx, None)
        else:
            _PINNED[self.idx] = self.prev


class Engine:
    def __init__(self, net: NetConfig, device="cuda"):
        self.lib = _ffi.lib()
        self.net = net
        self.device = torch.device(device)
        if self.device.type != "cuda":
            raise _ffi.IsdfError("isdf_amd kernels need a HIP device (got %s); there is no CPU path" % device)
        self.cnet = net.to_c()
        _ffi.check(self.lib.isdf_check_net(C.byref(self.cnet)),
                   "isdf_check_net(hidden=%d, blocks=%d, n_freqs=%d)" % (net.hidden, net.blocks, net.n_freqs))
        n = self.lib.isdf_param_count(C.byref(self.cnet))
        _ffi.check(min(n, 0), "isdf_param_count")
        self.n_params = int(n)
        self.params = torch.zeros(self.n_params, dtype=torch.float32, device=self.device)
        self.exp_avg = torch.zeros_like(self.params)
        self.exp_avg_sq = torch.zeros_like(self.params)
        sb = self.lib.isdf_shadow_bytes(C.byref(self.cnet))
        self.shadow = torch.zeros(int(sb), dtype=torch.uint8, device=self.device)
        self._ws = None
        self._ws_key = None
        self._scan_ws = None
        self.reduce_buf = None
        self.reduce_extra = 0
        self.reduce_floats = 0
        self.mailbox = None
        self._step_plans = {}
        self.opt_step = 0
        self.reduce_split = int(self.lib.isdf_reduce_split_floats(C.byref(self.cnet)))
        self.slices = {}
        off = 0
        for k, shp in net.param_shapes():
            cnt = int(np.prod(shp))
            self.slices[k] = (off, shp)
            off += cnt
        assert off == self.n_params

    def param_view(self, key):
        off, shp = self.slices[key]
        return self.params[off:off + int(np.prod(shp))].view(*shp)

    def load_params(self, state):
        for k, (off, shp) in self.slices.items():
            v = torch.as_tensor(np.asarray(state[k].detach().cpu() if torch.is_tensor(state[k]) else state[k]),
                                dtype=torch.float32).reshape(-1)
            self.params[off:off + v.numel()].copy_(v)
        self.pack()

    def pack(self):
        _ffi.check(self.lib.isdf_pack_weights(C.byref(self.cnet), _ffi.ptr(self.params),
                                              _ffi.ptr(self.shadow), _stream(self.device)), "isdf_pack_weights")

    def workspace(self, max_points, train):
        key = (int(max_points), bool(train))
        if self._ws is None or self._ws_key[0] < key[0] or (key[1] and not self._ws_key[1]):
            nb = self.lib.isdf_workspace_bytes(C.byref(self.cnet), int(max_points), int(train))
            _ffi.check(min(nb, 0), "isdf_workspace_bytes")
            self._ws = torch.empty(int(nb), dtype=torch.uint8, device=self.device)
            self._ws_key = key
        return self._ws

    def sample(self, depth_batch, T_WC_batch, normal_batch, frame_idx, normal_idx, sc: SampleConfig,
               draws=None, seed=0, offset=0, want_T=False, reuse=False):
        dev = self.device
        inline = isinstance(frame_idx, (tuple, list))
        if inline and (len(frame_idx) > _ffi.MAX_INLINE_FRAMES or
                       (normal_batch is not None and (normal_idx is None or len(normal_idx) != len(frame_idx)))):
            raise ValueError("inline windows hold up to %d keyframes (with one normal index each)" % _ffi.MAX_INLINE_FRAMES)
        F = len(frame_idx) if inline else int(frame_idx.numel())
        R0 = F * sc.n_rays
        S = sc.S
        key = (R0, S, bool(want_T), normal_batch is not None)
        slot = None
        if reuse:
            ring = getattr(self, "_smp_ring", None)
            if ring is None or ring[0] != key:
                ring = self._smp_ring = [key, [None, None], 0, [None, None]]
                self._step_plans.clear()
            ring[2] ^= 1
            slot = ring[2]
            plan = ring[3][slot]
            pkey = (depth_batch.data_ptr(), T_WC_batch.data_ptr(), 0 if normal_batch is None else normal_batch.data_ptr(),
                    -1 if inline else frame_idx.data_ptr(),
                    -1 if inline else (0 if normal_idx is None else normal_idx.data_ptr()), sc.n_rays, sc.H, sc.W,
                    sc.fx, sc.fy, sc.cx, sc.cy, sc.n_strat, sc.n_surf, sc.min_depth, sc.dist_behind_surf)
            if draws is None and plan is not None and plan[0] == pkey:
                _, a, o, out = plan
                a.seed, a.offset = int(seed), int(offset)
                if inline:
                    a.frame_idx_inline[:F] = frame_idx
                    if normal_idx is not None:
                        a.normal_idx_inline[:F] = normal_idx
                _ffi.check(self.lib.isdf_sample_rays(C.byref(a), C.byref(o), self._scan_ptr, self._scan_ws.numel(),
                                                     _stream(self.device)), "isdf_sample_rays")
                return dict(out)
        a = _ffi.SampleArgs()
        a.depth_batch, a.T_WC_batch = depth_batch.data_ptr(), T_WC_batch.data_ptr()
        a.normal_batch = None if normal_batch is None else normal_batch.data_ptr()
        if inline:
            a.n_inline = F
            a.frame_idx_inline[:F] = [int(v) for v in frame_idx]
            if normal_idx is not None:
                a.normal_idx_inline[:F] = [int(v) for v in normal_idx]
        else:
            a.frame_idx = frame_idx.data_ptr()
            a.normal_idx = None if normal_idx is None else normal_idx.data_ptr()
        a.n_frames, a.n_rays, a.H, a.W = F, sc.n_rays, sc.H, sc.W
        a.fx, a.fy, a.cx, a.cy = sc.fx, sc.fy, sc.cx, sc.cy
        a.n_strat, a.n_surf = sc.n_strat, sc.n_surf
        a.min_depth, a.dist_behind_surf = sc.min_depth, sc.dist_behind_surf
        keep = []
        if draws is not None:
            a.rng_mode = 0
            for name, dkey, dt in (("draw_h", "indices_h", torch.int64), ("draw_w", "indices_w", torch.int64),
                                   ("draw_u", "U", torch.float32), ("draw_n", "N_off", torch.float32)):
                t = draws.get(dkey)
                if t is not None:
                    t = t.to(device=dev, dtype=dt).contiguous()
                    keep.append(t)
                    setattr(a, name, t.data_ptr())
        else:
            a.rng_mode = 1
            a.seed, a.offset = int(seed), int(offset)
        out = self._smp_ring[1][slot] if slot is not None else None
        if out is None:
            e = lambda *shape, dt=torch.float32: torch.empty(*shape, dtype=dt, device=dev)
            out = dict(
                n_valid=e(1, dt=torch.int32),
                indices_b=e(R0, dt=torch.int64), indices_h=e(R0, dt=torch.int64), indices_w=e(R0, dt=torch.int64),
                depth_sample=e(R0), dirs_C_sample=e(R0, 3),
                norm_sample=None if normal_batch is None else e(R0, 3),
                T_WC_sample=e(R0, 4, 4) if want_T else None,
                dirs_W_sample=e(R0, 3), z_vals=e(R0, S), pc=e(R0, S, 3))
            if slot is not None:
                self._smp_ring[1][slot] = out
        out = dict(out)
        o = _ffi.SampleOut()
        for k, v in out.items():
            setattr(o, k, None if v is None else v.data_ptr())
        need = int(self.lib.isdf_sample_scan_bytes(R0))
        if self._scan_ws is None or self._scan_ws.numel() < need:
            self._scan_ws = torch.zeros(max(need, 4096), dtype=torch.uint8, device=dev)
            if getattr(self, "_smp_ring", None) is not None:
                self._smp_ring[3] = [None, None]
        self._scan_ptr = _ffi.ptr(self._scan_ws)
        _ffi.check(self.lib.isdf_sample_rays(C.byref(a), C.byref(o), self._scan_ptr, self._scan_ws.numel(),
                                             _stream(self.device)), "isdf_sample_rays")
        out["max_rays"] = R0
        out["S"] = S
        out["n_frames"] = F
        out["_keep"] = keep
        if slot is not None and draws is None:
            out["_slot"] = slot
            self._smp_ring[3][slot] = (pkey, a, o, dict(out))
        return out

    def sdf_eval(self, pts, noise=None, want_grad=False):
        shp = pts.shape[:-1]
        x = pts.reshape(-1, 3).to(device=self.device, dtype=torch.float32).contiguous()
        n = x.shape[0]
        sdf = torch.empty(n, dtype=torch.float32, device=self.device)
        grad = torch.empty(n, 3, dtype=torch.float32, device=self.device) if want_grad else None
        ws = self.workspace(n, False) if want_grad else None
        nz = None if noise is None else noise.reshape(-1).to(device=self.device, dtype=torch.float32).contiguous()
        _ffi.check(self.lib.isdf_sdf_eval(C.byref(self.cnet), _ffi.ptr(self.params), _ffi.ptr(self.shadow),
                                          _ffi.ptr(x), n, _ffi.ptr(nz), _ffi.ptr(sdf), _ffi.ptr(grad),
                                          _ffi.ptr(ws), 0 if ws is None else ws.numel(), _stream(self.device)),
                   "isdf_sdf_eval")
        if want_grad:
            return sdf.view(*shp), grad.view(*shp, 3)
        return sdf.view(*shp)

    def train_step(self, smp, lc: LossConfig, sc: SampleConfig, noise=None, debug=False, prof_events=None,
                   noise_std=0.0, noise_seed=0, noise_offset=0, optim=None, surf_group=None, extra_slot=0, extra_value=0.0,
                   split_event=None):
        dev = self.device
        F, R0, S = smp["n_frames"], smp["max_rays"], smp["S"]
        plan_key = None
        if (smp.get("_slot") is not None and noise is None and not debug and surf_group is None
                and lc.bounds_method == "ray"):
            fo = None if optim is None else optim.get("frame_avg_out")
            fi = None if optim is None else optim.get("frame_avg_index")
            fi_inline = isinstance(fi, (tuple, list))
            ns = smp.get("norm_sample")
            plan_key = (smp["_slot"], smp["pc"].data_ptr(), smp["n_valid"].data_ptr(), smp["indices_b"].data_ptr(),
                        smp["z_vals"].data_ptr(), 0 if ns is None else ns.data_ptr(),
                        R0, S, F, sc.H, sc.W, lc.loss_type, lc.trunc_weight, lc.trunc_distance,
                        lc.eik_weight, lc.eik_apply_dist, lc.grad_weight, lc.orien_loss, optim is None,
                        0 if fo is None else fo.data_ptr(), 0 if fi is None else (-1 if fi_inline else fi.data_ptr()), self.reduce_extra,
                        0 if split_event is None else split_event.cuda_event,
                        None if self.reduce_buf is None else self.reduce_buf.data_ptr(), None if self._ws is None else self._ws.data_ptr())
            plan = self._step_plans.get(smp["_slot"])
            if plan is not None and plan[0] == plan_key:
                _, closs, a, o, q, ws, dbg = plan
                a.noise_std, a.noise_seed, a.noise_offset = float(noise_std), int(noise_seed), int(noise_offset)
                a.extra_slot, a.extra_value = int(extra_slot), float(extra_value)
                o.prof_events = prof_events
                if q is not None:
                    self.opt_step += 1
                    betas = optim.get("betas", (0.9, 0.999))
                    q.lr, q.weight_decay = float(optim.get("lr", 0.0013)), float(optim.get("weight_decay", 0.012))
                    q.beta1, q.beta2, q.eps = float(betas[0]), float(betas[1]), float(optim.get("eps", 1e-8))
                    q.grad_scale, q.step = float(optim.get("grad_scale", 1.0)), int(self.opt_step)
                    if fi_inline:
                        q.frame_avg_index_inline[:F] = fi
                    _ffi.check(self.lib.isdf_train_step_adamw(C.byref(self.cnet), C.byref(closs), C.byref(a), C.byref(o),
                                                              C.byref(q), self._ws_ptr, ws.numel(), _stream(self.device)),
                               "isdf_train_step_adamw")
                else:
                    _ffi.check(self.lib.isdf_train_step(C.byref(self.cnet), C.byref(closs), self._params_ptr, self._shadow_ptr,
                                                        C.byref(a), C.byref(o), self._ws_ptr, ws.numel(), _stream(self.device)),
                               "isdf_train_step")
                return dict(dbg)
        nred = int(self.lib.isdf_reduce_floats(C.byref(self.cnet), F))
        if self.reduce_buf is None or self.reduce_buf.numel() != nred + self.reduce_extra:
            self.reduce_buf = torch.zeros(nred + self.reduce_extra, dtype=torch.float32, device=dev)
        self.reduce_floats = nred
        if self.mailbox is None or self.mailbox.numel() != 8 + self.reduce_extra:
            self.mailbox = torch.zeros(8 + self.reduce_extra, dtype=torch.float32, pin_memory=True)
        ws = self.workspace(R0 * S, True)
        self._ws_ptr, self._params_ptr, self._shadow_ptr = _ffi.ptr(ws), _ffi.ptr(self.params), _ffi.ptr(self.shadow)
        closs = lc.to_c()
        a = _ffi.StepArgs()
        a.n_valid = smp["n_valid"].data_ptr()
        a.max_rays, a.S, a.n_frames, a.H, a.W = R0, S, F, sc.H, sc.W
        for k in ("pc", "z_vals", "depth_sample", "dirs_C_sample", "dirs_W_sample", "indices_b",
                  "indices_h", "indices_w"):
            setattr(a, k, smp[k].data_ptr())
        a.norm_sample = None if smp.get("norm_sample") is None else smp["norm_sample"].data_ptr()
        keep = []
        a.noise_std, a.noise_seed, a.noise_offset = float(noise_std), int(noise_seed), int(noise_offset)
        a.extra_floats, a.extra_slot, a.extra_value = int(self.reduce_extra), int(extra_slot), float(extra_value)
        if noise is not None:
            if (noise.numel() == R0 * S and noise.dtype == torch.float32 and noise.device == dev
                    and noise.is_contiguous()):
                nz = noise
            else:
                nz = torch.zeros(R0 * S, dtype=torch.float32, device=dev)
                nn_ = noise.reshape(-1).to(device=dev, dtype=torch.float32)
                nz[:nn_.numel()] = nn_
            keep.append(nz)
            a.noise = nz.data_ptr()
        if lc.bounds_method == "pc":
            pb = torch.empty(R0 * S, dtype=torch.float32, device=dev)
            pg = torch.empty(R0 * S, 3, dtype=torch.float32, device=dev)
            surf = None
            if surf_group is not None:
                from . import dp
                surf = dp.gather_surface_points(smp["pc"], smp["n_valid"], surf_group)
                keep.append(surf)
            _ffi.check(self.lib.isdf_bounds_pc(_ffi.ptr(smp["n_valid"]), R0, S, _ffi.ptr(smp["pc"]),
                                               _ffi.ptr(smp["z_vals"]), _ffi.ptr(smp["depth_sample"]),
                                               _ffi.ptr(surf), 0 if surf is None else surf.shape[0],
                                               _ffi.ptr(pb), _ffi.ptr(pg), _stream(self.device)), "isdf_bounds_pc")
            a.pc_bounds, a.pc_grad_vec = pb.data_ptr(), pg.data_ptr()
            keep += [pb, pg]
        o = _ffi.StepOut()
        o.reduce_buf = self.reduce_buf.data_ptr()
        o.host_mailbox = self.mailbox.data_ptr()
        if prof_events is not None:
            o.prof_events = prof_events
        if split_event is not None:
            if optim is not None:
                raise ValueError("split_event belongs to the two-call (data-parallel) form")
            o.split_event = split_event.cuda_event
        dbg = {}
        if debug:
            dbg = dict(sdf=torch.zeros(R0, S, device=dev), sdf_grad=torch.zeros(R0, S, 3, device=dev),
                       tot_loss_mat=torch.zeros(R0, S, device=dev))
            o.sdf, o.sdf_grad, o.tot_loss_mat = (dbg["sdf"].data_ptr(), dbg["sdf_grad"].data_ptr(),
                                                 dbg["tot_loss_mat"].data_ptr())
            if lc.bounds_method == "pc":
                dbg["pc_bounds"], dbg["pc_grad_vec"] = keep[-2].view(R0, S), keep[-1].view(R0, S, 3)
        if optim is not None:
            q = self._optim_args(optim, F, dbg, keep)
            _ffi.check(self.lib.isdf_train_step_adamw(C.byref(self.cnet), C.byref(closs), C.byref(a), C.byref(o),
                                                      C.byref(q), _ffi.ptr(ws), ws.numel(), _stream(self.device)),
                       "isdf_train_step_adamw")
        else:
            _ffi.check(self.lib.isdf_train_step(C.byref(self.cnet), C.byref(closs), _ffi.ptr(self.params),
                                                _ffi.ptr(self.shadow), C.byref(a), C.byref(o), _ffi.ptr(ws),
                                                ws.numel(), _stream(self.device)), "isdf_train_step")
        dbg["_keep"] = keep
        if plan_key is not None:
            plan_key = plan_key[:-2] + (self.reduce_buf.data_ptr(), self._ws.data_ptr())
            self._step_plans[smp["_slot"]] = (plan_key, closs, a, o, q if optim is not None else None, ws, dbg)
        return dbg

    def _optim_args(self, optim, F, dbg, keep):
        self.opt_step += 1
        betas = optim.get("betas", (0.9, 0.999))
        q = _ffi.OptimArgs()
        q.params, q.exp_avg, q.exp_avg_sq = self.params.data_ptr(), self.exp_avg.data_ptr(), self.exp_avg_sq.data_ptr()
        q.shadow = self.shadow.data_ptr()
        q.lr, q.weight_decay = float(optim.get("lr", 0.0013)), float(optim.get("weight_decay", 0.012))
        q.beta1, q.beta2, q.eps = float(betas[0]), float(betas[1]), float(optim.get("eps", 1e-8))
        q.grad_scale, q.step = float(optim.get("grad_scale", 1.0)), int(self.opt_step)
        if optim.get("frame_avg_out") is not None:
            la = torch.empty(F, 8, 8, dtype=torch.float32, device=self.device)
            fa_out, fa_idx = optim["frame_avg_out"], optim.get("frame_avg_index")
            assert fa_out.dtype == torch.float32 and fa_out.is_contiguous()
            q.loss_approx, q.frame_avg = la.data_ptr(), fa_out.data_ptr()
            if isinstance(fa_idx, (tuple, list)):
                assert len(fa_idx) == F <= _ffi.MAX_INLINE_FRAMES
                q.frame_avg_inline_n = F
                q.frame_avg_index_inline[:F] = [int(v) for v in fa_idx]
            else:
                assert fa_idx is None or (fa_idx.dtype == torch.int32 and fa_idx.numel() == F)
                q.frame_avg_index = None if fa_idx is None else fa_idx.data_ptr()
            dbg["loss_approx"] = la
            keep += [fa_out, fa_idx]
        return q

    def allreduce_direct(self, rccl):
        fn, comm = rccl
        _ffi.check(self.lib.isdf_allreduce_sum_f32(fn, comm, _ffi.ptr(self.reduce_buf), int(self.reduce_buf.numel()),
                                                   _stream(self.device)), "isdf_allreduce_sum_f32")

    def train_step_finish(self, n_frames, optim):
        dbg, keep = {}, []
        fo, fi = optim.get("frame_avg_out"), optim.get("frame_avg_index")
        fi_inline = isinstance(fi, (tuple, list))
        fkey = (n_frames, 0 if fo is None else fo.data_ptr(), 0 if fi is None else (-1 if fi_inline else fi.data_ptr()),
                self.reduce_buf.data_ptr(), self.mailbox.data_ptr(), self.reduce_extra)
        plan = self._step_plans.get("finish")
        if plan is not None and plan[0] == fkey:
            _, q, dbg = plan
            self.opt_step += 1
            betas = optim.get("betas", (0.9, 0.999))
            q.lr, q.weight_decay = float(optim.get("lr", 0.0013)), float(optim.get("weight_decay", 0.012))
            q.beta1, q.beta2, q.eps = float(betas[0]), float(betas[1]), float(optim.get("eps", 1e-8))
            q.grad_scale, q.step = float(optim.get("grad_scale", 1.0)), int(self.opt_step)
            if fi_inline:
                q.frame_avg_index_inline[:n_frames] = fi
        else:
            q = self._optim_args(optim, n_frames, dbg, keep)
            dbg["_keep"] = keep
            self._step_plans["finish"] = (fkey, q, dbg)
        _ffi.check(self.lib.isdf_train_step_finish(C.byref(self.cnet), C.byref(q), _ffi.ptr(self.reduce_buf), int(n_frames),
                                                   int(self.reduce_extra), _ffi.ptr(self.mailbox), _stream(self.device)),
                   "isdf_train_step_finish")
        dbg["_keep"] = keep
        return dbg

    def grad_view(self, key):
        off, shp = self.slices[key]
        return self.reduce_buf[off:off + int(np.prod(shp))].view(*shp)

    def loss_sums(self):
        return self.reduce_buf[self.n_params:self.n_params + 8]

    def frame_avg(self, n_frames, out=None, index=None):
        if isinstance(index, (tuple, list)):
            key = tuple(int(v) for v in index)
            cache = self.__dict__.setdefault("_fa_index_cache", {})
            if key not in cache:
                if len(cache) > 64:
                    cache.clear()
                cache[key] = torch.as_tensor(key, dtype=torch.int32, device=self.device)
            index = cache[key]
        la = torch.empty(n_frames, 8, 8, dtype=torch.float32, device=self.device)
        if out is None:
            fa = torch.empty(n_frames, dtype=torch.float32, device=self.device)
        else:
            assert out.dtype == torch.float32 and out.is_contiguous()
            assert index is None or (index.dtype == torch.int32 and index.numel() == n_frames)
            fa = out
        _ffi.check(self.lib.isdf_frame_avg(_ffi.ptr(self.reduce_buf), self.n_params, n_frames, _ffi.ptr(la),
                                           _ffi.ptr(fa), _ffi.ptr(index), _stream(self.device)), "isdf_frame_avg")
        return la, fa

    def estimate_normals(self, depth, sc: "SampleConfig"):
        d = depth.to(device=self.device, dtype=torch.float32).contiguous()
        out = torch.empty(d.shape[0], d.shape[1], 3, dtype=torch.float32, device=self.device)
        _ffi.check(self.lib.isdf_estimate_normals(_ffi.ptr(d), d.shape[0], d.shape[1], sc.fx, sc.fy, sc.cx, sc.cy,
                                                  _ffi.ptr(out), _stream(self.device)), "isdf_estimate_normals")
        return out

    def render_depth(self, z_vals, sdf, depth_sample=None, kf_dist_th=0.1, n_valid=None):
        R, S = z_vals.shape
        view = torch.zeros(R, dtype=torch.float32, device=self.device)
        below = torch.zeros(1, dtype=torch.int32, device=self.device)
        _ffi.check(self.lib.isdf_render_depth(_ffi.ptr(n_valid), R, R, S, _ffi.ptr(z_vals.contiguous()),
                                              _ffi.ptr(sdf.contiguous()), _ffi.ptr(depth_sample), float(kf_dist_th),
                                              _ffi.ptr(view), _ffi.ptr(below), _stream(self.device)), "isdf_render_depth")
        return view, below

    def adamw(self, lr=0.0013, weight_decay=0.012, betas=(0.9, 0.999), eps=1e-8, grad_scale=1.0,
              use_device_count=True):
        self.opt_step += 1
        cnt = self.reduce_buf[self.n_params + _ffi.LS_COUNT:] if use_device_count else None
        _ffi.check(self.lib.isdf_adamw(C.byref(self.cnet), _ffi.ptr(self.params), _ffi.ptr(self.exp_avg),
                                       _ffi.ptr(self.exp_avg_sq), _ffi.ptr(self.reduce_buf), _ffi.ptr(cnt),
                                       float(grad_scale), float(lr), float(betas[0]), float(betas[1]),
                                       float(eps), float(weight_decay), int(self.opt_step),
                                       _ffi.ptr(self.shadow), _stream(self.device)), "isdf_adamw")
```

### isdf_amd/hot_path.py

```python
import copy
import ctypes
import os
import sys
import types

import numpy as np
import torch

from . import _ffi, dp, frame_store
from .engine import LossConfig, NetConfig, SampleConfig
from .modules import PositionalEncodingHIP, SDFMapHIP


class FlatAdamW:

    def __init__(self, sdf_map, lr, weight_decay, betas=(0.9, 0.999), eps=1e-8):
        self.sdf_map = sdf_map
        self.param_groups = [dict(params=list(sdf_map.parameters()), lr=lr, betas=betas, eps=eps,
                                  weight_decay=weight_decay, amsgrad=False)]

    def step(self):
        g = self.param_groups[0]
        self.sdf_map.engine.adamw(lr=g["lr"], weight_decay=g["weight_decay"], betas=g["betas"], eps=g["eps"])

    def zero_grad(self, set_to_none=True):
        pass

    def state_dict(self):
        eng = self.sdf_map.engine
        state = {}
        if eng.opt_step > 0:
            for i, (k, (off, shp)) in enumerate(eng.slices.items()):
                n = int(np.prod(shp))
                state[i] = dict(step=torch.tensor(float(eng.opt_step)),
                                exp_avg=eng.exp_avg[off:off + n].view(*shp).clone(),
                                exp_avg_sq=eng.exp_avg_sq[off:off + n].view(*shp).clone())
        g = dict(self.param_groups[0])
        g["params"] = list(range(len(eng.slices)))
        return dict(state=state, param_groups=[g])

    def load_state_dict(self, sd):
        eng = self.sdf_map.engine
        if not sd["state"]:
            eng.exp_avg.zero_(); eng.exp_avg_sq.zero_(); eng.opt_step = 0
        for i, (k, (off, shp)) in enumerate(eng.slices.items()):
            if i in sd["state"]:
                n = int(np.prod(shp))
                eng.exp_avg[off:off + n].copy_(sd["state"][i]["exp_avg"].reshape(-1))
                eng.exp_avg_sq[off:off + n].copy_(sd["state"][i]["exp_avg_sq"].reshape(-1))
                eng.opt_step = int(float(sd["state"][i]["step"]))
        for k in ("lr", "weight_decay", "betas", "eps"):
            if sd.get("param_groups") and k in sd["param_groups"][0]:
                self.param_groups[0][k] = sd["param_groups"][0][k]


_CUDA_GET_DEVICE = getattr(torch._C, "_cuda_getDevice", None)


class StepLosses(dict):

    def __init__(self, loss_sums_host, has_grad, has_eik):
        ls = loss_sums_host.tolist()
        n = max(ls[_ffi.LS_COUNT], 1.0)
        super().__init__()
        self["sdf_loss"] = ls[_ffi.LS_SDF] / n
        if has_grad:
            self["grad_loss"] = ls[_ffi.LS_GRAD] / n
        if has_eik:
            self["eikonal_loss"] = ls[_ffi.LS_EIK] / n
        self["total_loss"] = torch.scalar_tensor(ls[_ffi.LS_TOTAL] / n)


class _LazyCut(dict):

    def __init__(self, raw):
        super().__init__()
        self._raw = raw

    def _fill(self):
        if self._raw is not None:
            R = int(self._raw["n_valid"].item())
            for k in ("indices_b", "indices_h", "indices_w"):
                dict.__setitem__(self, k, self._raw[k][:R])
            self._raw = None

    def __getitem__(self, k):
        self._fill(); return dict.__getitem__(self, k)

    def keys(self):
        self._fill(); return dict.keys(self)

    def items(self):
        self._fill(); return dict.items(self)

    def values(self):
        self._fill(); return dict.values(self)

    def __iter__(self):
        self._fill(); return dict.__iter__(self)

    def __len__(self):
        return 3

    def __contains__(self, k):
        return k in ("indices_b", "indices_h", "indices_w")


class _BackwardDone(torch.autograd.Function):

    @staticmethod
    def forward(ctx, value, anchor):
        return value.clone()

    @staticmethod
    def backward(ctx, g):
        return None, None


class HotPath:

    def _loss_cfg(self):
        return LossConfig(self.bounds_method, self.loss_type, self.trunc_weight, self.trunc_distance,
                          self.eik_weight, self.eik_apply_dist, self.grad_weight, bool(self.orien_loss))

    def _sample_cfg(self, n_rays=None, dist_behind_surf=None, n_strat=None, n_surf=None):
        return SampleConfig(n_rays=self.n_rays if n_rays is None else n_rays,
                            n_strat=self.n_strat_samples if n_strat is None else n_strat,
                            n_surf=self.n_surf_samples if n_surf is None else n_surf,
                            min_depth=self.min_depth,
                            dist_behind_surf=self.dist_behind_surf if dist_behind_surf is None else dist_behind_surf,
                            H=self.H, W=self.W, fx=self.fx, fy=self.fy, cx=self.cx, cy=self.cy)

    @property
    def engine(self):
        return self.sdf_map.engine

    def _rank(self):
        g = self._hip.dist_group
        return 0 if g is None else torch.distributed.get_rank(g)

    def _draws_torch(self, F, sc, n_valid_fn):
        dev = self._hip.device
        total = sc.n_rays * F
        ih = torch.randint(0, sc.H, (total,), device=dev)
        iw = torch.randint(0, sc.W, (total,), device=dev)
        R = n_valid_fn(ih, iw)
        U = torch.rand(R, sc.n_strat, device=dev)
        N_off = torch.normal(torch.zeros(R, max(sc.n_surf - 1, 0)), 0.1).to(dev)
        return dict(indices_h=ih, indices_w=iw, U=U, N_off=N_off)

    def _sample_raw(self, depth_batch, T_WC_batch, norm_batch, frame_idx, normal_idx, sc, want_T, shared_key=False,
                    reuse=False):
        eng, hip = self.engine, self._hip
        if hip.rng == "torch":
            as_t = lambda ix: torch.as_tensor(list(ix), dtype=torch.long, device=hip.device) if isinstance(ix, (tuple, list)) else ix.long()
            fi_t, ni_t = as_t(frame_idx), (None if normal_idx is None else as_t(normal_idx))

            def n_valid(ih, iw):
                ib = torch.arange(fi_t.numel(), device=ih.device).repeat_interleave(sc.n_rays)
                d = depth_batch[fi_t[ib], ih, iw]
                ok = d != 0
                if norm_batch is not None:
                    ok &= ~torch.isnan(norm_batch[ni_t[ib], ih, iw, 0])
                return int(ok.sum().item())
            draws = self._draws_torch(fi_t.numel(), sc, n_valid)
            return eng.sample(depth_batch, T_WC_batch, norm_batch, frame_idx, normal_idx, sc, draws=draws,
                              want_T=want_T, reuse=reuse)
        hip.draw_count += 1
        seed = hip.seed if shared_key else dp.rank_seed(hip.seed, self._rank())
        return eng.sample(depth_batch, T_WC_batch, norm_batch, frame_idx, normal_idx, sc,
                          seed=seed, offset=hip.draw_count, want_T=want_T, reuse=reuse)

    def sample_points(self, depth_batch, T_WC_batch, norm_batch=None, active_loss_approx=None, n_rays=None,
                      dist_behind_surf=None, n_strat_samples=None, n_surf_samples=None, _shared_key=False):
        if active_loss_approx is not None:
            raise Exception('Active sampling not currently supported.')
        sc = self._sample_cfg(n_rays, dist_behind_surf, n_strat_samples, n_surf_samples)
        dev = self._hip.device
        ar = torch.arange(depth_batch.shape[0], dtype=torch.int32, device=dev)
        s = self._sample_raw(depth_batch.contiguous(), T_WC_batch.contiguous(),
                             None if norm_batch is None else norm_batch.contiguous(), ar,
                             None if norm_batch is None else ar, sc, want_T=True, shared_key=_shared_key)
        R = int(s["n_valid"].item())

        def cut(t):
            return None if t is None else t[:R]
        return {
            "depth_batch": depth_batch, "pc": cut(s["pc"]), "z_vals": cut(s["z_vals"]),
            "indices_b": cut(s["indices_b"]), "indices_h": cut(s["indices_h"]), "indices_w": cut(s["indices_w"]),
            "dirs_C_sample": cut(s["dirs_C_sample"]), "depth_sample": cut(s["depth_sample"]),
            "T_WC_sample": cut(s["T_WC_sample"]), "norm_sample": cut(s["norm_sample"]),
            "binary_masks": None,
            "_raw": s, "_sc": sc,
        }

    def _raw_from_public(self, sample):
        dev = self._hip.device
        pc = sample["pc"].detach().to(dev, torch.float32).contiguous()
        R, S = pc.shape[0], pc.shape[1]
        T = sample["T_WC_sample"].to(dev, torch.float32)
        dC = sample["dirs_C_sample"].to(dev, torch.float32).contiguous()
        dW = (T[:, :3, :3] * dC[:, None, :]).sum(-1).contiguous()
        i64 = lambda t: t.to(dev, torch.int64).contiguous()
        F = int(sample["depth_batch"].shape[0])
        s = dict(n_valid=torch.tensor([R], dtype=torch.int32, device=dev), pc=pc,
                 z_vals=sample["z_vals"].to(dev, torch.float32).contiguous(),
                 depth_sample=sample["depth_sample"].to(dev, torch.float32).contiguous(),
                 dirs_C_sample=dC, dirs_W_sample=dW,
                 norm_sample=None if sample.get("norm_sample") is None else sample["norm_sample"].to(dev, torch.float32).contiguous(),
                 indices_b=i64(sample["indices_b"]), indices_h=i64(sample["indices_h"]), indices_w=i64(sample["indices_w"]),
                 max_rays=R, S=S, n_frames=F)
        sc = self._sample_cfg(n_strat=S - self.n_surf_samples)
        return s, sc

    def _step_kernels(self, s, sc, fused_optim, frame_avg_dst):
        hip, eng = self._hip, self.engine
        noise, kw = None, {}
        if self.noise_std is not None:
            if hip.rng == "torch":
                R = int(s["n_valid"].item())
                noise = torch.randn(R, s["S"], device=hip.device) * self.noise_std
            else:
                hip.noise_count += 1
                kw = dict(noise_std=self.noise_std, noise_seed=dp.rank_seed(hip.seed, self._rank()),
                          noise_offset=hip.noise_count)
        if fused_optim:
            g = self.optimiser.param_groups[0]
            kw["optim"] = dict(lr=g["lr"], weight_decay=g["weight_decay"], betas=g["betas"], eps=g["eps"])
            if frame_avg_dst is not None:
                kw["optim"].update(frame_avg_out=frame_avg_dst[0], frame_avg_index=frame_avg_dst[1])
        if hip.dist_group is not None and self.bounds_method == "pc":
            kw["surf_group"] = hip.dist_group
        if hip.clock_slots:
            kw.update(extra_slot=hip.rank, extra_value=hip.prev_step_ms)
        if hip.prof_events is not None:
            kw["prof_events"], hip.prof_events = hip.prof_events, None
        split = hip.dist_group is not None and hip.overlap_allreduce and not fused_optim
        if split:
            if hip.split_event is None:
                hip.split_event, hip.comm_stream = dp.new_split_event(hip.device), torch.cuda.Stream(hip.device)
            kw["split_event"] = hip.split_event
        dbg = eng.train_step(s, self._loss_cfg(), sc, noise=noise, **kw)
        if split:
            dp.allreduce_split_(eng.reduce_buf, eng.reduce_split, hip.split_event, hip.comm_stream, hip.dist_group)
        elif hip.dist_group is not None:
            if hip.rccl is not None:
                eng.allreduce_direct(hip.rccl)
            else:
                dp.allreduce_(eng.reduce_buf, hip.dist_group)
        return dbg

    def sdf_eval_and_loss(self, sample, do_avg_loss=True):
        if "_raw" in sample:
            s, sc = sample["_raw"], sample["_sc"]
        else:
            s, sc = self._raw_from_public(sample)
        self._step_kernels(s, sc, fused_optim=False, frame_avg_dst=None)
        eng = self.engine
        ls = eng.loss_sums().detach().cpu()
        losses = StepLosses(ls, self.grad_weight != 0, self.eik_weight != 0)
        anchor = next(iter(self.sdf_map.parameters()))
        total_loss = _BackwardDone.apply((eng.loss_sums()[_ffi.LS_TOTAL] / eng.loss_sums()[_ffi.LS_COUNT]).detach(), anchor)
        loss_approx = frame_avg_loss = None
        if do_avg_loss:
            loss_approx, frame_avg_loss = eng.frame_avg(s["n_frames"])
        return total_loss, losses, loss_approx, frame_avg_loss

    def _timing_start(self, st):
        if st is not None:
            st.synchronize()
            ev = self._hip.timing_events
            if ev is None:
                ev = self._hip.timing_events = (torch.cuda.Event(enable_timing=True), torch.cuda.Event(enable_timing=True))
            ev[0].record(st)
            return ev
        import time
        return time.perf_counter(), None

    def _timing_end(self, st, start, end):
        if st is not None:
            end.record(st)
            st.synchronize()
            return start.elapsed_time(end)
        import time
        return (time.perf_counter() - start) * 1000.0

    def step(self):
        dev = self._hip.device
        if dev.type != "cuda":
            return self._step(None)
        from .engine import pinned_stream
        if _CUDA_GET_DEVICE is not None and dev.index is not None and _CUDA_GET_DEVICE() == dev.index:
            with pinned_stream(dev.index) as st:
                return self._step(st)
        with torch.cuda.device(dev), pinned_stream(dev) as st:
            return self._step(st)

    def _step(self, st):
        hip = self._hip
        start, end = self._timing_start(st)

        K = self.frames.T_WC_batch.shape[0]
        if len(self.frames) > self.window_size and self.incremental:
            if hip.device.type == "cuda" and self.frames.frame_avg_losses.device.type == "cuda":
                to_host = getattr(self.frames, "losses_to_host", None)
                if to_host is not None:
                    to_host()
            idxs = self._select_window()
        else:
            idxs = np.arange(K)
        self.active_idxs = idxs
        if hip.inline_window and len(idxs) <= _ffi.MAX_INLINE_FRAMES:
            fidx = tuple(idxs.tolist()) if isinstance(idxs, np.ndarray) else tuple(int(i) for i in idxs)
            nidx = fidx if hip.fix_normal_window else tuple(range(len(fidx)))
        else:
            key = (tuple(int(i) for i in idxs), bool(hip.fix_normal_window))
            if hip.idx_cache is None or hip.idx_cache[0] != key:
                fidx = torch.as_tensor(np.asarray(idxs), dtype=torch.int32, device=hip.device)
                nidx = fidx if hip.fix_normal_window else torch.arange(len(idxs), dtype=torch.int32, device=hip.device)
                hip.idx_cache = (key, fidx, nidx)
            _, fidx, nidx = hip.idx_cache
        norm_batch = self.frames.normal_batch if self.do_normal else None
        sc = self._sample_cfg()
        s = self._sample_raw(self.frames.depth_batch, self.frames.T_WC_batch, norm_batch, fidx,
                             nidx if norm_batch is not None else None, sc, want_T=False, reuse=True)
        self.active_pixels = _LazyCut(s)

        fal = self.frames.frame_avg_losses
        fused = hip.dist_group is None and hip.fuse_optimiser
        direct = fal.is_contiguous() and fal.dtype == torch.float32 and (fal.device == hip.device or self._pinned(fal))
        dbg = self._step_kernels(s, sc, fused, (fal, fidx) if direct else None)
        eng = self.engine
        if not fused and direct and hip.fuse_optimiser:
            g = self.optimiser.param_groups[0]
            eng.train_step_finish(len(idxs), dict(lr=g["lr"], weight_decay=g["weight_decay"], betas=g["betas"], eps=g["eps"],
                                                  frame_avg_out=fal, frame_avg_index=fidx))
        else:
            if not fused or not direct:
                if direct:
                    eng.frame_avg(len(idxs), out=fal, index=fidx)
                else:
                    _, fa = eng.frame_avg(len(idxs))
                    self.frames.frame_avg_losses[[int(i) for i in idxs]] = fa
            if not fused:
                self.optimiser.step()
        if getattr(eng, "mailbox", None) is None:
            hip.loss_host.copy_(eng.loss_sums(), non_blocking=True)
            mailbox = hip.loss_host
        else:
            mailbox = eng.mailbox
            if hip.dist_group is not None and not (not fused and direct and hip.fuse_optimiser):
                mailbox[:8].copy_(eng.loss_sums(), non_blocking=True)
                if hip.clock_slots:
                    mailbox[8:].copy_(eng.reduce_buf[eng.reduce_floats:], non_blocking=True)

        step_time = self._timing_end(st, start, end)
        clock_ms = step_time
        if hip.virtual_step_ms is not None:
            clock_ms = step_time = float(hip.virtual_step_ms)
        elif hip.clock_slots:
            clock_ms = float(mailbox[8:8 + hip.clock_slots].max()) if mailbox.numel() >= 8 + hip.clock_slots else \
                float(eng.reduce_buf[eng.reduce_floats:].max())
            hip.prev_step_ms = float(np.float32(step_time))
        losses = StepLosses(mailbox, self.grad_weight != 0, self.eik_weight != 0)
        hip.step_count += 1
        self.tot_step_time += (1 / self.frac_time_perception) * (clock_ms / 1000.0)
        self.steps_since_frame += 1
        return losses, step_time

    def _pinned(self, t):
        hip = self._hip
        if t.device.type != "cpu" or hip.device.type != "cuda":
            return False
        key = (t.data_ptr(), t.numel())
        if getattr(hip, "pinned_key", None) != key:
            hip.pinned_key, hip.pinned_ok = key, bool(t.is_pinned())
        return hip.pinned_ok

    def _select_window(self):
        hip = self._hip
        if hip.dist_group is None:
            return self.select_keyframes()
        saved = np.random.get_state()
        np.random.set_state(hip.window_rng_state)
        try:
            return self.select_keyframes()
        finally:
            hip.window_rng_state = np.random.get_state()
            np.random.set_state(saved)

    def is_keyframe(self, T_WC, depth_gt):
        hip = self._hip
        sample_pts = self.sample_points(depth_gt, T_WC, n_rays=self.n_rays_is_kf, dist_behind_surf=0.8,
                                        _shared_key=hip.dist_group is not None)
        s = sample_pts["_raw"]
        pc = s["pc"]
        n = int(sample_pts["pc"].shape[0])
        noise = None
        if self.noise_std is not None:
            noise = torch.zeros(pc.shape[:-1], device=hip.device)
            noise[:n] = torch.randn(n, pc.shape[1], device=hip.device) * self.noise_std
        sdf = self.frozen_sdf_map.engine.sdf_eval(pc, noise=noise)
        view, below = self.engine.render_depth(s["z_vals"], sdf, s["depth_sample"], self.kf_dist_th,
                                               n_valid=s["n_valid"])
        below_th_prop = float(below.item()) / n if n > 0 else float("nan")
        is_keyframe = below_th_prop < self.kf_pixel_ratio
        print("Proportion of loss below threshold", below_th_prop, "for KF should be less than",
              self.kf_pixel_ratio, " ---> is keyframe:", is_keyframe)
        return is_keyframe

    def get_data(self, idxs):
        geo = self._hip.geometry_transform
        if not self.do_normal or geo is None:
            return super().get_data(idxs)
        eng, hip = self.engine, self._hip

        class _DepthAsPointCloud:
            def __init__(self, depth, fx, fy, cx, cy):
                self.depth, self.k = depth, (fx, fy, cx, cy)

        def pointcloud_from_depth(depth, fx, fy, cx, cy):
            return _DepthAsPointCloud(depth, fx, fy, cx, cy)

        def estimate_normals(pc):
            if not isinstance(pc, _DepthAsPointCloud):
                return saved[1](pc)
            fx, fy, cx, cy = pc.k
            hip.ingest_launches += 1
            return eng.estimate_normals(pc.depth, SampleConfig(H=int(pc.depth.shape[0]), W=int(pc.depth.shape[1]),
                                                               fx=float(fx), fy=float(fy), cx=float(cx), cy=float(cy)))
        saved = (geo.pointcloud_from_depth_torch, geo.estimate_pointcloud_normals)
        geo.pointcloud_from_depth_torch, geo.estimate_pointcloud_normals = pointcloud_from_depth, estimate_normals
        try:
            return super().get_data(idxs)
        finally:
            geo.pointcloud_from_depth_torch, geo.estimate_pointcloud_normals = saved

    def check_keyframe_latest(self):
        add_new_frame = super().check_keyframe_latest()
        hip = self._hip
        if hip.dist_group is not None:
            v = dp.broadcast_floats([float(add_new_frame), float(self.last_is_keyframe), float(self.optim_frames),
                                     -1.0 if self.noise_std is None else float(self.noise_std)], hip.dist_group, hip.device)
            add_new_frame, self.last_is_keyframe, self.optim_frames = bool(v[0]), bool(v[1]), int(v[2])
            self.noise_std = None if v[3] < 0 else v[3]
        return add_new_frame

    def add_frame(self, frame_data):
        hip = self._hip
        if hip.dist_group is not None:
            for k in ("depth_batch", "T_WC_batch", "normal_batch"):
                t = getattr(frame_data, k, None)
                if torch.is_tensor(t):
                    torch.distributed.broadcast(t, dp.src_rank(hip.dist_group), group=hip.dist_group)
        return super().add_frame(frame_data)

    def hip_state_dict(self):
        fr, hip = self.frames, self._hip
        frozen = getattr(self, "frozen_sdf_map", None)
        return {
            "model_state_dict": {k: v.detach().clone() for k, v in self.sdf_map.state_dict().items()},
            "optimizer_state_dict": self.optimiser.state_dict(),
            "frozen_state_dict": None if frozen is None else {k: v.detach().clone() for k, v in frozen.state_dict().items()},
            "frames": {k: (None if getattr(fr, k, None) is None else
                           (getattr(fr, k).copy() if isinstance(getattr(fr, k), np.ndarray) else
                            (getattr(fr, k).clone() if torch.is_tensor(getattr(fr, k)) else copy.deepcopy(getattr(fr, k)))))
                       for k in FRAME_FIELDS if hasattr(fr, k)},
            "clock": dict(tot_step_time=self.tot_step_time, steps_since_frame=self.steps_since_frame,
                          last_is_keyframe=self.last_is_keyframe, optim_frames=self.optim_frames,
                          noise_std=self.noise_std, step_count=hip.step_count,
                          prev_step_ms=hip.prev_step_ms),
            "rng": dict(draw_count=hip.draw_count, noise_count=hip.noise_count, seed=hip.seed,
                        window=getattr(hip, "window_rng_state", None),
                        numpy=np.random.get_state(), torch=torch.get_rng_state(),
                        torch_cuda=torch.cuda.get_rng_state(hip.device) if hip.device.type == "cuda" else None),
        }

    def load_hip_state_dict(self, sd):
        hip = self._hip
        self.sdf_map.load_state_dict(sd["model_state_dict"])
        self.optimiser.load_state_dict(sd["optimizer_state_dict"])
        if sd.get("frozen_state_dict") is not None:
            self.frozen_sdf_map = copy.deepcopy(self.sdf_map)
            self.frozen_sdf_map.load_state_dict(sd["frozen_state_dict"])
        f = sd["frames"]
        fr = type(self.frames)()
        for k, v in f.items():
            setattr(fr, k, v)
        for twin, src in (("im_batch_np", "im_batch"), ("depth_batch_np", "depth_batch"), ("T_WC_batch_np", "T_WC_batch")):
            if twin not in f and getattr(fr, src, None) is not None and hasattr(fr, twin):
                t = getattr(fr, src).detach()
                if twin == "im_batch_np":
                    t = (t * 255).round().to(torch.uint8)
                setattr(fr, twin, t.cpu().numpy())
        fal = getattr(fr, "frame_avg_losses", None)
        if fal is not None and fal.device.type == "cpu" and hip.device.type == "cuda" and not fal.is_pinned():
            fr.frame_avg_losses = fal.pin_memory()
        self.frames = fr
        c = sd["clock"]
        self.tot_step_time, self.steps_since_frame = c["tot_step_time"], c["steps_since_frame"]
        self.last_is_keyframe, self.optim_frames = c["last_is_keyframe"], c["optim_frames"]
        self.noise_std, hip.step_count = c["noise_std"], c["step_count"]
        hip.prev_step_ms = float(c.get("prev_step_ms", 0.0))
        r = sd["rng"]
        hip.draw_count, hip.noise_count, hip.seed = r["draw_count"], r["noise_count"], r["seed"]
        hip.idx_cache = None
        if r.get("window") is not None:
            hip.window_rng_state = r["window"]
        np.random.set_state(r["numpy"]); torch.set_rng_state(r["torch"])
        if r.get("torch_cuda") is not None:
            torch.cuda.set_rng_state(r["torch_cuda"], hip.device)


FRAME_FIELDS = ("frame_id", "im_batch", "im_batch_np", "depth_batch", "depth_batch_np", "T_WC_batch", "T_WC_batch_np",
                "normal_batch", "frame_avg_losses", "T_WC_track", "T_WC_gt", "count")

ENGINE_FACTORY = None


UNSUPPORTED_HINT = ("isdf_amd hot path: %s (the reference's own Python path is the CPU / fallback path; "
                    "this build ships no second implementation)")


def unsupported_reason(trainer):
    if getattr(trainer, "bounds_method", "ray") not in ("ray", "pc"):
        return "bounds_method %r (only 'ray' and 'pc' can run upstream, loss.py:29)" % (trainer.bounds_method,)
    if getattr(trainer, "do_active", False):
        return "active sampling (rejected by the reference itself, trainer.py:718)"
    if getattr(trainer, "loss_type", "L1") not in ("L1", "L2"):
        return "loss_type %r (loss.py:104)" % (trainer.loss_type,)
    net = getattr(trainer, "sdf_map", None)
    if net is not None and not isinstance(net, SDFMapHIP) and ENGINE_FACTORY is None and os.path.exists(_ffi.LIB_PATH):
        try:
            pe = net.positional_encoding
            c = NetConfig(hidden=net.out_alpha.in_features, blocks=len(net.mid1), n_freqs=int(pe.n_freqs)).to_c()
        except AttributeError:
            return "trainer.sdf_map is not an isdf.modules.fc_map.SDFMap"
        rc = _ffi.lib().isdf_check_net(ctypes.byref(c))
        if rc != 0:
            return "network shape (hidden %d, %d blocks, %d octaves): %s" % (c.hidden, c.blocks, c.n_freqs,
                                                                              _ffi.lib().isdf_error_string(int(rc)).decode())
    return None


def can_graft(trainer):
    if unsupported_reason(trainer) is not None:
        return False
    if ENGINE_FACTORY is not None:
        return True
    return torch.device(trainer.device).type == "cuda" and torch.cuda.is_available() and os.path.exists(_ffi.LIB_PATH)


def graft(trainer, rng="philox", seed=1, dist_group=None, fix_normal_window=False, fwd_operand="fp16x2",
          fuse_optimiser=True, virtual_step_ms=None, engine_factory=None, overlap_allreduce=False, bwd_operand=None, spill_operand=None, migrate_frames=True):
    if isinstance(trainer, HotPath) and getattr(trainer, "_hip", None) is not None:
        return trainer
    if engine_factory is None:
        engine_factory = ENGINE_FACTORY
    dev = torch.device(trainer.device)
    if dev.type == "cuda" and dev.index is None and torch.cuda.is_available():
        dev = torch.device("cuda", torch.cuda.current_device())
    if engine_factory is None and dev.type != "cuda":
        raise _ffi.IsdfError(UNSUPPORTED_HINT % ("device %r is not a HIP device" % (trainer.device,)))
    why = unsupported_reason(trainer)
    if why is not None:
        raise _ffi.IsdfError(UNSUPPORTED_HINT % why)
    if rng not in ("philox", "torch"):
        raise ValueError("rng must be 'philox' or 'torch'")

    old = getattr(trainer, "sdf_map", None)
    if old is not None and not isinstance(old, SDFMapHIP):
        pe_old = old.positional_encoding
        pe = PositionalEncodingHIP(min_deg=pe_old.min_deg, max_deg=pe_old.max_deg, scale=pe_old.scale,
                                   transform=pe_old.transform)
        n_block = len(old.mid1)
        hidden = old.out_alpha.in_features
        with torch.random.fork_rng(devices=[]):
            new = SDFMapHIP(pe, hidden_size=hidden, hidden_layers_block=n_block, scale_output=old.scale_output,
                            device=dev, fwd_operand=fwd_operand, engine_factory=engine_factory,
                            bwd_operand=bwd_operand, spill_operand=spill_operand)
        new.load_state_dict({k: v.detach() for k, v in old.state_dict().items()})
        new.train(old.training)
        trainer.sdf_map = new
        og = trainer.optimiser.param_groups[0]
        old_state = trainer.optimiser.state_dict()
        trainer.optimiser = FlatAdamW(new, lr=og["lr"], weight_decay=og["weight_decay"], betas=tuple(og["betas"]),
                                      eps=og["eps"])
        if old_state.get("state"):
            trainer.optimiser.load_state_dict(old_state)
        if getattr(trainer, "frozen_sdf_map", None) is not None:
            fz = copy.deepcopy(new)
            fz.load_state_dict({k: v.detach() for k, v in trainer.frozen_sdf_map.state_dict().items()})
            trainer.frozen_sdf_map = fz
    elif old is None:
        raise ValueError("graft() needs a trainer whose load_networks() has run")

    hip = types.SimpleNamespace(rng=rng, seed=int(seed), dist_group=dist_group, fix_normal_window=bool(fix_normal_window),
                                fuse_optimiser=bool(fuse_optimiser), device=dev, draw_count=0, noise_count=0,
                                step_count=0, idx_cache=None, timing_events=None, prof_events=None,
                                inline_window=True,
                                overlap_allreduce=bool(overlap_allreduce) and dist_group is not None, split_event=None,
                                comm_stream=None,
                                virtual_step_ms=None if virtual_step_ms is None else float(virtual_step_ms),
                                loss_host=torch.zeros(8, dtype=torch.float32,
                                                      pin_memory=(dev.type == "cuda")))
    geo = getattr(getattr(sys.modules.get(trainer.__class__.__module__), "geometry", None), "transform", None)
    hip.geometry_transform = geo if (geo is not None and hasattr(geo, "pointcloud_from_depth_torch")
                                     and hasattr(geo, "estimate_pointcloud_normals")) else None
    hip.ingest_launches = 0
    if migrate_frames and getattr(trainer, "frames", None) is not None and not isinstance(trainer.frames, frame_store.FrameData):
        trainer.frames = frame_store.FrameData.from_reference(trainer.frames)
    trainer._hip = hip
    base = trainer.__class__
    if not issubclass(base, HotPath):
        trainer.__class__ = type("Hip" + base.__name__, (HotPath, base), {"__module__": HotPath.__module__})
    hip.clock_slots, hip.prev_step_ms, hip.rank, hip.rccl, hip.collective = 0, 0.0, 0, None, None
    if dist_group is not None:
        eng = trainer.sdf_map.engine
        for t in (eng.params, eng.exp_avg, eng.exp_avg_sq):
            torch.distributed.broadcast(t, dp.src_rank(dist_group), group=dist_group)
        eng.pack()
        hip.rank, hip.world = torch.distributed.get_rank(dist_group), torch.distributed.get_world_size(dist_group)
        hip.window_rng_state = np.random.RandomState(hip.seed + 104729).get_state()
        if hip.virtual_step_ms is None:
            hip.clock_slots = eng.reduce_extra = hip.world
        if hasattr(eng, "allreduce_direct") and hip.device.type == "cuda":
            from .engine import _stream
            hip.rccl = dp.rccl_agree(eng.lib, dp.rccl_direct(dist_group, hip.device), dist_group, hip.device, _stream(hip.device))
        hip.collective = "rccl on the step's stream (isdf_allreduce_sum_f32)" if hip.rccl is not None else "torch.distributed.all_reduce"
    return trainer
```

Baseline: 3956 train-steps/s.

## Add native single-call train step with device-published completion and host spin-wait

```diff
diff --git a/include/isdf_hip.h b/include/isdf_hip.h
--- a/include/isdf_hip.h
+++ b/include/isdf_hip.h
@@ -8,7 +8,7 @@
 extern "C" {
 #endif
 
-#define ISDF_ABI_VERSION 7
+#define ISDF_ABI_VERSION 8
 
 enum {
   ISDF_OK = 0,
@@ -165,6 +165,52 @@
                           const isdf_step_out* o, const isdf_optim_args* opt, void* workspace,
                           int64_t workspace_bytes, void* stream);
 
+typedef struct isdf_step_done {
+  uint64_t t_start;
+  uint64_t t_end;
+  uint32_t seq;
+  uint32_t reserved;
+} isdf_step_done;
+
+typedef struct isdf_step_plan {
+  const isdf_net_cfg* net;
+  const isdf_loss_cfg* loss;
+  isdf_sample_args* sample_args;
+  const isdf_sample_out* sample_out;
+  void* scan_ws;
+  int64_t scan_ws_bytes;
+  isdf_step_args* step_args;
+  const isdf_step_out* step_out;
+  isdf_optim_args* optim_args;
+  void* workspace;
+  int64_t workspace_bytes;
+  void* sync_ws;
+  isdf_step_done* done;
+  int32_t wall_clock_khz;
+  uint32_t seq;
+} isdf_step_plan;
+
+typedef struct isdf_step_scalars {
+  float lr, beta1, beta2, eps, weight_decay, grad_scale;
+  int32_t step;
+  int32_t n_frames;
+  uint64_t seed, offset;
+  float noise_std;
+  int32_t spin_budget_us;
+  uint64_t noise_seed, noise_offset;
+  int32_t frame_idx[8];
+  int32_t normal_idx[8];
+} isdf_step_scalars;
+
+typedef struct isdf_step_result {
+  float step_ms;
+  uint32_t seq;
+  int32_t slept;
+  int32_t reserved;
+} isdf_step_result;
+
+int isdf_train_step_sync(isdf_step_plan* plan, const isdf_step_scalars* s, isdf_step_result* r, void* stream);
+
 int isdf_train_step_finish(const isdf_net_cfg* net, const isdf_optim_args* opt, const float* reduce_buf,
                            int32_t n_frames, int32_t extra_floats, float* host_mailbox, void* stream);
 
diff --git a/isdf_amd/_ffi.py b/isdf_amd/_ffi.py
--- a/isdf_amd/_ffi.py
+++ b/isdf_amd/_ffi.py
@@ -4,7 +4,7 @@
 HERE = os.path.dirname(os.path.abspath(__file__))
 LIB_PATH = os.environ.get("ISDF_HIP_LIB") or os.path.join(HERE, "libisdf_hip.so")
 
-ABI_VERSION = 7
+ABI_VERSION = 8
 
 SYMBOLS = [
     "isdf_abi_version", "isdf_error_string", "isdf_check_net", "isdf_param_count", "isdf_shadow_bytes",
@@ -12,6 +12,7 @@
     "isdf_sample_rays",
     "isdf_sdf_eval", "isdf_train_step", "isdf_train_step_adamw", "isdf_train_step_finish", "isdf_bounds_pc",
     "isdf_frame_avg", "isdf_adamw", "isdf_estimate_normals", "isdf_render_depth", "isdf_allreduce_sum_f32",
+    "isdf_train_step_sync",
 ]
 
 LS_SDF, LS_GRAD, LS_EIK, LS_TOTAL, LS_COUNT = 0, 1, 2, 3, 4
@@ -78,6 +79,29 @@
 MAX_INLINE_FRAMES = 8
 
 
+class StepDone(C.Structure):
+    _fields_ = [("t_start", C.c_uint64), ("t_end", C.c_uint64), ("seq", C.c_uint32), ("reserved", C.c_uint32)]
+
+
+class StepPlan(C.Structure):
+    _fields_ = [("net", C.POINTER(NetCfg)), ("loss", C.POINTER(LossCfg)), ("sample_args", C.POINTER(SampleArgs)),
+                ("sample_out", C.POINTER(SampleOut)), ("scan_ws", C.c_void_p), ("scan_ws_bytes", C.c_int64),
+                ("step_args", C.POINTER(StepArgs)), ("step_out", C.POINTER(StepOut)), ("optim_args", C.POINTER(OptimArgs)),
+                ("workspace", C.c_void_p), ("workspace_bytes", C.c_int64), ("sync_ws", C.c_void_p), ("done", C.c_void_p),
+                ("wall_clock_khz", C.c_int32), ("seq", C.c_uint32)]
+
+
+class StepScalars(C.Structure):
+    _fields_ = [("lr", C.c_float), ("beta1", C.c_float), ("beta2", C.c_float), ("eps", C.c_float), ("weight_decay", C.c_float),
+                ("grad_scale", C.c_float), ("step", C.c_int32), ("n_frames", C.c_int32), ("seed", C.c_uint64),
+                ("offset", C.c_uint64), ("noise_std", C.c_float), ("spin_budget_us", C.c_int32), ("noise_seed", C.c_uint64),
+                ("noise_offset", C.c_uint64), ("frame_idx", C.c_int32 * 8), ("normal_idx", C.c_int32 * 8)]
+
+
+class StepResult(C.Structure):
+    _fields_ = [("step_ms", C.c_float), ("seq", C.c_uint32), ("slept", C.c_int32), ("reserved", C.c_int32)]
+
+
 
 class IsdfError(RuntimeError):
     pass
@@ -122,6 +146,7 @@
     L.isdf_adamw.argtypes = [P(NetCfg), vp, vp, vp, vp, vp, f32, f32, f32, f32, f32, f32, i32, vp, vp]
     L.isdf_estimate_normals.argtypes = [vp, i32, i32, f32, f32, f32, f32, vp, vp]
     L.isdf_render_depth.argtypes = [vp, i64, i64, i32, vp, vp, vp, f32, vp, vp, vp]
+    L.isdf_train_step_sync.argtypes = [P(StepPlan), P(StepScalars), P(StepResult), vp]
     for n in SYMBOLS[SYMBOLS.index("isdf_pack_weights"):]:
         getattr(L, n).restype = C.c_int
     if L.isdf_abi_version() != ABI_VERSION:
diff --git a/isdf_amd/csrc/capi.hip b/isdf_amd/csrc/capi.hip
--- a/isdf_amd/csrc/capi.hip
+++ b/isdf_amd/csrc/capi.hip
@@ -1,3 +1,4 @@
+#include <chrono>
 #include <cstdio>
 #include "isdf_common.h"
 #include "chain_params.h"
@@ -7,7 +8,8 @@
 namespace isdf {
 int launch_chain(const ChainParams& p, int mode, int64_t nTiles, hipStream_t st);
 int launch_dw(const DwParams& p, hipStream_t st);
-int launch_sample_rays(const isdf_sample_args& a, const isdf_sample_out& o, void* scan_ws, hipStream_t st);
+int launch_sample_rays(const isdf_sample_args& a, const isdf_sample_out& o, void* scan_ws, hipStream_t st,
+                       unsigned long long* t_stamp = nullptr);
 int64_t sample_scan_bytes(int64_t max_rays);
 int launch_adamw(float* p, float* m, float* v, const float* g, const float* cnt, float gs, float lr, float b1,
                  float b2, float eps, float wd, int step, int64_t n, hipStream_t st);
@@ -24,7 +26,7 @@
                      const float* tot_ws, const int64_t* ib, const int64_t* ih, const int64_t* iw, int F, int H, int W,
                      float* loss_sums, float* bl, float* bc, float* la_out, float* fa_out, const int32_t* fa_index,
                      hipStream_t st, float* mailbox, float* extra, int n_extra, int extra_slot, float extra_value, int part = 0,
-                     int fa_inline_n = 0, const int32_t* fa_inline = nullptr);
+                     int fa_inline_n = 0, const int32_t* fa_inline = nullptr, const StepSync* sync = nullptr);
 int launch_frame_avg(const float* bl, const float* bc, int F, float* la, float* fa, const int32_t* fa_index,
                      hipStream_t st);
 int launch_bounds_pc(const int32_t* n_valid, int max_rays, int S, const float* pc, const float* z, const float* depth,
@@ -110,9 +112,8 @@
 
 int64_t isdf_sample_scan_bytes(int64_t max_rays) { return max_rays < 1 ? ISDF_EINVAL : sample_scan_bytes(max_rays); }
 
-int isdf_sample_rays(const isdf_sample_args* a, const isdf_sample_out* o, void* scan_ws, int64_t scan_ws_bytes,
-                     void* stream) {
-  isdf_clear_stale_hip_error();
+static int sample_rays_impl(const isdf_sample_args* a, const isdf_sample_out* o, void* scan_ws, int64_t scan_ws_bytes,
+                            void* stream, unsigned long long* t_stamp) {
   if (!a || !o || !a->depth_batch || !a->T_WC_batch || !o->n_valid || !o->indices_b ||
       !o->indices_h || !o->indices_w || !o->depth_sample || !o->dirs_C_sample || !o->dirs_W_sample || !o->z_vals ||
       !o->pc)
@@ -125,7 +126,13 @@
   if ((int64_t)a->n_frames * a->n_rays > 0x7fffffff / 64) return ISDF_EINVAL;
   if (a->rng_mode == 0 && (!a->draw_h || !a->draw_w || !a->draw_u || (a->n_surf > 1 && !a->draw_n))) return ISDF_EINVAL;
   if (!scan_ws || scan_ws_bytes < sample_scan_bytes((int64_t)a->n_frames * a->n_rays)) return ISDF_EWORKSPACE;
-  return launch_sample_rays(*a, *o, scan_ws, (hipStream_t)stream);
+  return launch_sample_rays(*a, *o, scan_ws, (hipStream_t)stream, t_stamp);
+}
+
+int isdf_sample_rays(const isdf_sample_args* a, const isdf_sample_out* o, void* scan_ws, int64_t scan_ws_bytes,
+                     void* stream) {
+  isdf_clear_stale_hip_error();
+  return sample_rays_impl(a, o, scan_ws, scan_ws_bytes, stream, nullptr);
 }
 
 int isdf_sdf_eval(const isdf_net_cfg* net, const float* params, const void* shadow, const float* pts,
@@ -152,8 +159,7 @@
 
 static int train_step_impl(const isdf_net_cfg* net, const isdf_loss_cfg* loss, const float* params, const void* shadow,
                            const isdf_step_args* a, const isdf_step_out* o, void* workspace, int64_t workspace_bytes,
-                           void* stream, const isdf_optim_args* opt) {
-  isdf_clear_stale_hip_error();
+                           void* stream, const isdf_optim_args* opt, const StepSync* sync = nullptr) {
   NetLayout l; int rc = make_layout(net, &l);
   if (rc) return rc;
   if (!layout_supported(l)) return ISDF_EUNSUPPORTED;
@@ -212,7 +218,7 @@
                           opt->weight_decay, opt->step, wgLoss, w.nTiles, a->n_valid, a->S, totLoss, a->indices_b,
                           a->indices_h, a->indices_w, a->n_frames, a->H, a->W, lossSums, blockLoss, blockCnt,
                           opt->loss_approx, opt->frame_avg, opt->frame_avg_index, st, o->host_mailbox, extra, a->extra_floats,
-                          a->extra_slot, a->extra_value, 0, opt->frame_avg_inline_n, opt->frame_avg_index_inline);
+                          a->extra_slot, a->extra_value, 0, opt->frame_avg_inline_n, opt->frame_avg_index_inline, sync);
     if (rc) return rc;
     if (ev && hipEventRecord(ev[3], st) != hipSuccess) return ISDF_EHIP;
     return ISDF_OK;
@@ -233,20 +239,121 @@
 int isdf_train_step(const isdf_net_cfg* net, const isdf_loss_cfg* loss, const float* params,
                     const void* shadow, const isdf_step_args* a, const isdf_step_out* o,
                     void* workspace, int64_t workspace_bytes, void* stream) {
+  isdf_clear_stale_hip_error();
   return train_step_impl(net, loss, params, shadow, a, o, workspace, workspace_bytes, stream, nullptr);
+}
+
+static int check_fused_optim(const isdf_step_args* a, const isdf_step_out* o, const isdf_optim_args* opt) {
+  if (!a || !opt || !opt->params || !opt->exp_avg || !opt->exp_avg_sq || !opt->shadow || opt->step < 1) return ISDF_EINVAL;
+  if ((opt->loss_approx == nullptr) != (opt->frame_avg == nullptr)) return ISDF_EINVAL;
+  if (opt->frame_avg_inline_n != 0 && (opt->frame_avg_inline_n != a->n_frames || opt->frame_avg_inline_n > ISDF_MAX_INLINE_FRAMES))
+    return ISDF_EINVAL;
+  for (int f = 0; f < opt->frame_avg_inline_n; ++f)
+    if (opt->frame_avg_index_inline[f] < 0) return ISDF_EINVAL;
+  if (o && o->split_event) return ISDF_EINVAL;
+  return ISDF_OK;
 }
 
 int isdf_train_step_adamw(const isdf_net_cfg* net, const isdf_loss_cfg* loss, const isdf_step_args* a,
                           const isdf_step_out* o, const isdf_optim_args* opt, void* workspace,
                           int64_t workspace_bytes, void* stream) {
-  if (!a || !opt || !opt->params || !opt->exp_avg || !opt->exp_avg_sq || !opt->shadow || opt->step < 1) return ISDF_EINVAL;
-  if ((opt->loss_approx == nullptr) != (opt->frame_avg == nullptr)) return ISDF_EINVAL;
-  if (opt->frame_avg_inline_n != 0 && (opt->frame_avg_inline_n != a->n_frames || opt->frame_avg_inline_n > ISDF_MAX_INLINE_FRAMES))
-    return ISDF_EINVAL;
-  for (int f = 0; f < opt->frame_avg_inline_n; ++f)
-    if (opt->frame_avg_index_inline[f] < 0) return ISDF_EINVAL;
-  if (o && o->split_event) return ISDF_EINVAL;
+  isdf_clear_stale_hip_error();
+  const int rc = check_fused_optim(a, o, opt);
+  if (rc) return rc;
   return train_step_impl(net, loss, opt->params, opt->shadow, a, o, workspace, workspace_bytes, stream, opt);
+}
+
+static inline void cpu_relax() {
+#if defined(__x86_64__) || defined(__i386__)
+  __builtin_ia32_pause();
+#elif defined(__aarch64__)
+  asm volatile("yield");
+#endif
+}
+
+static int hip_failed(hipError_t e) { g_isdf_last_hip_error = (int)e; return ISDF_EHIP; }
+
+int isdf_train_step_sync(isdf_step_plan* plan, const isdf_step_scalars* s, isdf_step_result* r, void* stream) {
+  isdf_clear_stale_hip_error();
+  if (!plan || !s || !r || !plan->net || !plan->loss || !plan->sample_args || !plan->sample_out || !plan->step_args ||
+      !plan->step_out || !plan->optim_args || !plan->workspace || !plan->sync_ws || !plan->done)
+    return ISDF_EINVAL;
+  isdf_sample_args* a = plan->sample_args;
+  isdf_step_args* sa = plan->step_args;
+  isdf_optim_args* q = plan->optim_args;
+  const int F = s->n_frames;
+  if (F < 1 || F > ISDF_MAX_INLINE_FRAMES || a->n_inline != F || a->n_frames != F || sa->n_frames != F ||
+      q->frame_avg_inline_n != F || !q->frame_avg || a->rng_mode != 1)
+    return ISDF_EINVAL;
+  if (plan->loss->bounds_method != 0 || sa->noise || plan->step_out->split_event) return ISDF_EINVAL;
+  for (int f = 0; f < F; ++f)
+    if (s->frame_idx[f] < 0 || s->normal_idx[f] < 0) return ISDF_EINVAL;
+  if (plan->wall_clock_khz <= 0) {
+    int dev = 0, khz = 0;
+    hipError_t e = hipGetDevice(&dev);
+    if (e == hipSuccess) e = hipDeviceGetAttribute(&khz, hipDeviceAttributeWallClockRate, dev);
+    if (e != hipSuccess) return hip_failed(e);
+    if (khz <= 0) return ISDF_EUNSUPPORTED;
+    plan->wall_clock_khz = khz;
+  }
+  a->seed = s->seed; a->offset = s->offset;
+  sa->noise_std = s->noise_std; sa->noise_seed = s->noise_seed; sa->noise_offset = s->noise_offset;
+  q->lr = s->lr; q->beta1 = s->beta1; q->beta2 = s->beta2; q->eps = s->eps; q->weight_decay = s->weight_decay;
+  q->grad_scale = s->grad_scale; q->step = s->step;
+  for (int f = 0; f < F; ++f) {
+    a->frame_idx_inline[f] = s->frame_idx[f];
+    a->normal_idx_inline[f] = s->normal_idx[f];
+    q->frame_avg_index_inline[f] = s->frame_idx[f];
+  }
+  int rc = check_fused_optim(sa, plan->step_out, q);
+  if (rc) return rc;
+  hipStream_t st = (hipStream_t)stream;
+  unsigned int* ctr = (unsigned int*)plan->sync_ws;
+  unsigned long long* t_start = (unsigned long long*)((char*)plan->sync_ws + 8);
+  const uint32_t seq = plan->seq + 1u;
+  rc = sample_rays_impl(a, plan->sample_out, plan->scan_ws, plan->scan_ws_bytes, stream, t_start);
+  if (rc) return rc;
+  const StepSync sync = {ctr, t_start, plan->done, seq};
+  rc = train_step_impl(plan->net, plan->loss, q->params, q->shadow, sa, plan->step_out, plan->workspace, plan->workspace_bytes,
+                       stream, q, &sync);
+  if (rc) return rc;
+  plan->seq = seq;
+
+  using clk = std::chrono::steady_clock;
+  const auto t0 = clk::now();
+  const auto budget = std::chrono::microseconds(s->spin_budget_us > 0 ? s->spin_budget_us : 50000);
+  auto nextQuery = t0 + std::chrono::microseconds(100);
+  r->slept = 0;
+  uint32_t seen = __atomic_load_n(&plan->done->seq, __ATOMIC_ACQUIRE);
+  while (seen != seq) {
+    cpu_relax();
+    seen = __atomic_load_n(&plan->done->seq, __ATOMIC_ACQUIRE);
+    if (seen == seq) break;
+    const auto now = clk::now();
+    if (now >= nextQuery) {
+      const hipError_t e = hipStreamQuery(st);
+      if (e != hipSuccess && e != hipErrorNotReady) return hip_failed(e);
+      nextQuery = now + std::chrono::microseconds(100);
+      if (e == hipSuccess) {
+        seen = __atomic_load_n(&plan->done->seq, __ATOMIC_ACQUIRE);
+        if (seen != seq) return hip_failed(hipErrorUnknown);
+        break;
+      }
+    }
+    if (now - t0 > budget) {
+      const hipError_t e = hipStreamSynchronize(st);
+      if (e != hipSuccess) return hip_failed(e);
+      r->slept = 1;
+      seen = __atomic_load_n(&plan->done->seq, __ATOMIC_ACQUIRE);
+      if (seen != seq) return hip_failed(hipErrorUnknown);
+      break;
+    }
+  }
+  const uint64_t ts = __atomic_load_n(&plan->done->t_start, __ATOMIC_RELAXED);
+  const uint64_t te = __atomic_load_n(&plan->done->t_end, __ATOMIC_RELAXED);
+  r->seq = seen;
+  r->step_ms = te >= ts ? (float)((double)(te - ts) / (double)plan->wall_clock_khz) : 0.f;
+  return ISDF_OK;
 }
 
 int isdf_train_step_finish(const isdf_net_cfg* net, const isdf_optim_args* opt, const float* reduce_buf, int32_t n_frames,
diff --git a/isdf_amd/csrc/isdf_common.h b/isdf_amd/csrc/isdf_common.h
--- a/isdf_amd/csrc/isdf_common.h
+++ b/isdf_amd/csrc/isdf_common.h
@@ -79,6 +79,14 @@
   return ISDF_EHIP;
 }
 #endif
+
+struct StepSync {
+  unsigned int* ctr;
+  const unsigned long long* t_start;
+  isdf_step_done* done;
+  uint32_t seq;
+};
+constexpr int SYNC_WS_BYTES = 64;
 
 inline int round_up(int x, int m) { return (x + m - 1) / m * m; }
 
diff --git a/isdf_amd/csrc/optim.hip b/isdf_amd/csrc/optim.hip
--- a/isdf_amd/csrc/optim.hip
+++ b/isdf_amd/csrc/optim.hip
@@ -197,6 +197,8 @@
   FinalizeArgs fin;
   int nW, nV;
   int wBlock0;
+  StepSync sync;
+  uint32_t nBlocks;
 };
 
 __device__ __forceinline__ void shadow_put(const NetLayout& L, uint16_t* sh, bool fwdSet, int64_t elem, float val,
@@ -225,8 +227,7 @@
 }
 
 template <int PHASE>
-__global__ __launch_bounds__(1024) void step_tail_kernel(const TailParams p) {
-  __shared__ FinalizeLds lds;
+__device__ __forceinline__ void step_tail_body(const TailParams& p, FinalizeLds& lds) {
   const NetLayout& L = p.lay;
   const int HD = L.HD;
   const int b = blockIdx.x;
@@ -339,6 +340,37 @@
   }
 }
 
+__device__ __forceinline__ void step_tail_publish(const TailParams& p, bool hostWriter) {
+  asm volatile("s_waitcnt vmcnt(0)" ::: "memory");
+  __syncthreads();
+  if (threadIdx.x != 0) return;
+  unsigned int old;
+  if (hostWriter) {
+    __builtin_amdgcn_fence(__ATOMIC_RELEASE, "");
+    asm volatile("s_waitcnt vmcnt(0)" ::: "memory");
+    old = __hip_atomic_fetch_add(p.sync.ctr, 1u, __ATOMIC_RELEASE, __HIP_MEMORY_SCOPE_SYSTEM);
+  } else {
+    old = __hip_atomic_fetch_add(p.sync.ctr, 1u, __ATOMIC_RELAXED, __HIP_MEMORY_SCOPE_AGENT);
+  }
+  if (old != p.nBlocks - 1) return;
+  __builtin_amdgcn_fence(__ATOMIC_ACQUIRE, "");
+  __hip_atomic_store(p.sync.ctr, 0u, __ATOMIC_RELAXED, __HIP_MEMORY_SCOPE_AGENT);
+  const unsigned long long t1 = __builtin_amdgcn_s_memrealtime();
+  const unsigned long long t0 = __hip_atomic_load(p.sync.t_start, __ATOMIC_RELAXED, __HIP_MEMORY_SCOPE_AGENT);
+  __hip_atomic_store(&p.sync.done->t_start, (uint64_t)t0, __ATOMIC_RELAXED, __HIP_MEMORY_SCOPE_SYSTEM);
+  __hip_atomic_store(&p.sync.done->t_end, (uint64_t)t1, __ATOMIC_RELAXED, __HIP_MEMORY_SCOPE_SYSTEM);
+  __builtin_amdgcn_fence(__ATOMIC_RELEASE, "");
+  asm volatile("s_waitcnt vmcnt(0)" ::: "memory");
+  __hip_atomic_store(&p.sync.done->seq, p.sync.seq, __ATOMIC_RELAXED, __HIP_MEMORY_SCOPE_SYSTEM);
+}
+
+template <int PHASE>
+__global__ __launch_bounds__(1024) void step_tail_kernel(const TailParams p) {
+  __shared__ FinalizeLds lds;
+  step_tail_body<PHASE>(p, lds);
+  if (PHASE == 0 && p.sync.done) step_tail_publish(p, (int)blockIdx.x >= p.nW + p.nV);
+}
+
 __global__ void frame_avg_kernel(const float* __restrict__ block_loss, const float* __restrict__ block_cnt,
                                  int n_frames, float* __restrict__ loss_approx, float* __restrict__ frame_avg,
                                  const int32_t* __restrict__ fa_index) {
@@ -409,7 +441,7 @@
                      const float* tot_ws, const int64_t* ib, const int64_t* ih, const int64_t* iw, int F, int H, int W,
                      float* loss_sums, float* bl, float* bc, float* la_out, float* fa_out, const int32_t* fa_index,
                      hipStream_t st, float* mailbox, float* extra, int n_extra, int extra_slot, float extra_value, int part,
-                     int fa_inline_n, const int32_t* fa_inline) {
+                     int fa_inline_n, const int32_t* fa_inline, const StepSync* sync) {
   TailParams p = {};
   p.lay = L; p.dwPart = dwPart; p.vecPart = vecPart; p.vecStride = vecStride; p.grad = grad;
   p.params = params; p.m = m; p.v = v; p.shadow = shadow; p.grad_scale = grad_scale;
@@ -436,6 +468,10 @@
   }
   const dim3 grid((unsigned)(p.nW + tailBlocks));
   if (grid.x == 0) return ISDF_OK;
+  if (sync) {
+    if (phase != 0 || part != 0) return ISDF_EINVAL;
+    p.sync = *sync; p.nBlocks = grid.x;
+  }
   if (phase == 0) hipLaunchKernelGGL(step_tail_kernel<0>, grid, dim3(1024), 0, st, p);
   else hipLaunchKernelGGL(step_tail_kernel<1>, grid, dim3(1024), 0, st, p);
   return isdf_launch_status();
diff --git a/isdf_amd/csrc/sampler.hip b/isdf_amd/csrc/sampler.hip
--- a/isdf_amd/csrc/sampler.hip
+++ b/isdf_amd/csrc/sampler.hip
@@ -43,7 +43,9 @@
 
 template <int CHUNK>
 __global__ __launch_bounds__(SMP_NT) void sample_rays_kernel(const isdf_sample_args a, const isdf_sample_out o,
-                                                              uint32_t* __restrict__ ws, int nChunks) {
+                                                              uint32_t* __restrict__ ws, int nChunks,
+                                                              unsigned long long* __restrict__ t_stamp) {
+  if (t_stamp && blockIdx.x == 0 && threadIdx.x == 0) *t_stamp = __builtin_amdgcn_s_memrealtime();
   constexpr bool SMALL = CHUNK == SMP_CHUNK_SMALL;
   constexpr int NT = SMP_NT, NW = NT / 64, GW = CHUNK / 64;
   __shared__ int sChunk, sBase;
@@ -258,14 +260,15 @@
 
 int64_t sample_scan_bytes(int64_t max_rays) { return 16 + 8 * ((max_rays + SMP_CHUNK_STREAM - 1) / SMP_CHUNK_STREAM); }
 
-int launch_sample_rays(const isdf_sample_args& a, const isdf_sample_out& o, void* scan_ws, hipStream_t st) {
+int launch_sample_rays(const isdf_sample_args& a, const isdf_sample_out& o, void* scan_ws, hipStream_t st,
+                       unsigned long long* t_stamp) {
   const int total = a.n_frames * a.n_rays;
   if (total <= SMP_SMALL_MAX_RAYS) {
     const int nChunks = (total + SMP_CHUNK_SMALL - 1) / SMP_CHUNK_SMALL;
-    hipLaunchKernelGGL(sample_rays_kernel<SMP_CHUNK_SMALL>, dim3((unsigned)nChunks), dim3(SMP_NT), 0, st, a, o, (uint32_t*)scan_ws, nChunks);
+    hipLaunchKernelGGL(sample_rays_kernel<SMP_CHUNK_SMALL>, dim3((unsigned)nChunks), dim3(SMP_NT), 0, st, a, o, (uint32_t*)scan_ws, nChunks, t_stamp);
   } else {
     const int nChunks = (total + SMP_CHUNK_STREAM - 1) / SMP_CHUNK_STREAM;
-    hipLaunchKernelGGL(sample_rays_kernel<SMP_CHUNK_STREAM>, dim3((unsigned)nChunks), dim3(SMP_NT), 0, st, a, o, (uint32_t*)scan_ws, nChunks);
+    hipLaunchKernelGGL(sample_rays_kernel<SMP_CHUNK_STREAM>, dim3((unsigned)nChunks), dim3(SMP_NT), 0, st, a, o, (uint32_t*)scan_ws, nChunks, t_stamp);
   }
   return isdf_launch_status();
 }
diff --git a/isdf_amd/engine.py b/isdf_amd/engine.py
--- a/isdf_amd/engine.py
+++ b/isdf_amd/engine.py
@@ -106,6 +106,7 @@
         return self.n_strat + self.n_surf
 
 
+_SYNC_WS_BYTES = 64
 _PINNED = {}
 
 
@@ -143,6 +144,13 @@
             _PINNED.pop(self.idx, None)
         else:
             _PINNED[self.idx] = self.prev
+
+
+def _sample_plan_key(depth_batch, T_WC_batch, normal_batch, frame_idx, normal_idx, sc, inline):
+    return (depth_batch.data_ptr(), T_WC_batch.data_ptr(), 0 if normal_batch is None else normal_batch.data_ptr(),
+            -1 if inline else frame_idx.data_ptr(),
+            -1 if inline else (0 if normal_idx is None else normal_idx.data_ptr()), sc.n_rays, sc.H, sc.W,
+            sc.fx, sc.fy, sc.cx, sc.cy, sc.n_strat, sc.n_surf, sc.min_depth, sc.dist_behind_surf)
 
 
 class Engine:
@@ -171,6 +179,12 @@
         self.reduce_floats = 0
         self.mailbox = None
         self._step_plans = {}
+        self._sync_plans = {}
+        self._sync_ws = self._done = None
+        self._sync_seq = 0
+        self._sync_scalars = _ffi.StepScalars()
+        self._sync_result = _ffi.StepResult()
+        self._sync_scalars_ref, self._sync_result_ref = C.byref(self._sync_scalars), C.byref(self._sync_result)
         self.opt_step = 0
         self.reduce_split = int(self.lib.isdf_reduce_split_floats(C.byref(self.cnet)))
         self.slices = {}
@@ -225,10 +239,7 @@
             ring[2] ^= 1
             slot = ring[2]
             plan = ring[3][slot]
-            pkey = (depth_batch.data_ptr(), T_WC_batch.data_ptr(), 0 if normal_batch is None else normal_batch.data_ptr(),
-                    -1 if inline else frame_idx.data_ptr(),
-                    -1 if inline else (0 if normal_idx is None else normal_idx.data_ptr()), sc.n_rays, sc.H, sc.W,
-                    sc.fx, sc.fy, sc.cx, sc.cy, sc.n_strat, sc.n_surf, sc.min_depth, sc.dist_behind_surf)
+            pkey = _sample_plan_key(depth_batch, T_WC_batch, normal_batch, frame_idx, normal_idx, sc, inline)
             if draws is None and plan is not None and plan[0] == pkey:
                 _, a, o, out = plan
                 a.seed, a.offset = int(seed), int(offset)
@@ -324,17 +335,9 @@
         plan_key = None
         if (smp.get("_slot") is not None and noise is None and not debug and surf_group is None
                 and lc.bounds_method == "ray"):
-            fo = None if optim is None else optim.get("frame_avg_out")
             fi = None if optim is None else optim.get("frame_avg_index")
             fi_inline = isinstance(fi, (tuple, list))
-            ns = smp.get("norm_sample")
-            plan_key = (smp["_slot"], smp["pc"].data_ptr(), smp["n_valid"].data_ptr(), smp["indices_b"].data_ptr(),
-                        smp["z_vals"].data_ptr(), 0 if ns is None else ns.data_ptr(),
-                        R0, S, F, sc.H, sc.W, lc.loss_type, lc.trunc_weight, lc.trunc_distance,
-                        lc.eik_weight, lc.eik_apply_dist, lc.grad_weight, lc.orien_loss, optim is None,
-                        0 if fo is None else fo.data_ptr(), 0 if fi is None else (-1 if fi_inline else fi.data_ptr()), self.reduce_extra,
-                        0 if split_event is None else split_event.cuda_event,
-                        None if self.reduce_buf is None else self.reduce_buf.data_ptr(), None if self._ws is None else self._ws.data_ptr())
+            plan_key = self._step_plan_key(smp, lc, sc, optim, split_event)
             plan = self._step_plans.get(smp["_slot"])
             if plan is not None and plan[0] == plan_key:
                 _, closs, a, o, q, ws, dbg = plan
@@ -432,6 +435,66 @@
             self._step_plans[smp["_slot"]] = (plan_key, closs, a, o, q if optim is not None else None, ws, dbg)
         return dbg
 
+    def _step_plan_key(self, smp, lc, sc, optim, split_event):
+        fo = None if optim is None else optim.get("frame_avg_out")
+        fi = None if optim is None else optim.get("frame_avg_index")
+        ns = smp.get("norm_sample")
+        return (smp["_slot"], smp["pc"].data_ptr(), smp["n_valid"].data_ptr(), smp["indices_b"].data_ptr(),
+                smp["z_vals"].data_ptr(), 0 if ns is None else ns.data_ptr(),
+                smp["max_rays"], smp["S"], smp["n_frames"], sc.H, sc.W, lc.loss_type, lc.trunc_weight, lc.trunc_distance,
+                lc.eik_weight, lc.eik_apply_dist, lc.grad_weight, lc.orien_loss, optim is None,
+                0 if fo is None else fo.data_ptr(), 0 if fi is None else (-1 if isinstance(fi, (tuple, list)) else fi.data_ptr()),
+                self.reduce_extra, 0 if split_event is None else split_event.cuda_event,
+                None if self.reduce_buf is None else self.reduce_buf.data_ptr(), None if self._ws is None else self._ws.data_ptr())
+
+    def train_step_sync(self, depth_batch, T_WC_batch, normal_batch, frame_idx, normal_idx, sc: SampleConfig, lc: LossConfig,
+                        seed, offset, optim, noise_std=0.0, noise_seed=0, noise_offset=0):
+        ring = getattr(self, "_smp_ring", None)
+        F = len(frame_idx)
+        if ring is None or ring[0] != (F * sc.n_rays, sc.S, False, normal_batch is not None) or self.mailbox is None:
+            return None
+        slot = ring[2] ^ 1
+        splan = ring[3][slot]
+        if splan is None or splan[0] != _sample_plan_key(depth_batch, T_WC_batch, normal_batch, frame_idx, normal_idx, sc, True):
+            return None
+        out = splan[3]
+        stplan = self._step_plans.get(slot)
+        if stplan is None or stplan[4] is None or stplan[0] != self._step_plan_key(out, lc, sc, optim, None):
+            return None
+        sp = self._sync_plans.get(slot)
+        if sp is None or sp[0] is not splan or sp[1] is not stplan:
+            if self._sync_ws is None:
+                self._sync_ws = torch.zeros(_SYNC_WS_BYTES, dtype=torch.uint8, device=self.device)
+                self._done = torch.zeros(C.sizeof(_ffi.StepDone), dtype=torch.uint8, pin_memory=True)
+            _, closs, sa, so, q, ws, _ = stplan
+            _, a, o, _ = splan
+            pl = _ffi.StepPlan()
+            pl.net, pl.loss = C.pointer(self.cnet), C.pointer(closs)
+            pl.sample_args, pl.sample_out = C.pointer(a), C.pointer(o)
+            pl.step_args, pl.step_out, pl.optim_args = C.pointer(sa), C.pointer(so), C.pointer(q)
+            pl.workspace, pl.workspace_bytes = ws.data_ptr(), ws.numel()
+            pl.sync_ws, pl.done = self._sync_ws.data_ptr(), self._done.data_ptr()
+            sp = self._sync_plans[slot] = (splan, stplan, pl, C.byref(pl))
+        pl = sp[2]
+        pl.scan_ws, pl.scan_ws_bytes = self._scan_ptr.value, self._scan_ws.numel()
+        pl.seq = self._sync_seq
+        stplan[3].prof_events = None
+        v = self._sync_scalars
+        betas = optim.get("betas", (0.9, 0.999))
+        v.lr, v.weight_decay = float(optim.get("lr", 0.0013)), float(optim.get("weight_decay", 0.012))
+        v.beta1, v.beta2, v.eps = float(betas[0]), float(betas[1]), float(optim.get("eps", 1e-8))
+        v.grad_scale, v.step, v.n_frames = float(optim.get("grad_scale", 1.0)), self.opt_step + 1, F
+        v.seed, v.offset = int(seed), int(offset)
+        v.noise_std, v.noise_seed, v.noise_offset = float(noise_std), int(noise_seed), int(noise_offset)
+        v.frame_idx[:F] = frame_idx
+        v.normal_idx[:F] = normal_idx
+        _ffi.check(self.lib.isdf_train_step_sync(sp[3], self._sync_scalars_ref, self._sync_result_ref, _stream(self.device)),
+                   "isdf_train_step_sync")
+        self._sync_seq = pl.seq
+        self.opt_step += 1
+        ring[2] = slot
+        return dict(out), self._sync_result.step_ms
+
     def _optim_args(self, optim, F, dbg, keep):
         self.opt_step += 1
         betas = optim.get("betas", (0.9, 0.999))
diff --git a/isdf_amd/hot_path.py b/isdf_amd/hot_path.py
--- a/isdf_amd/hot_path.py
+++ b/isdf_amd/hot_path.py
@@ -298,7 +298,11 @@
 
     def _step(self, st):
         hip = self._hip
-        start, end = self._timing_start(st)
+        native = (hip.step_path == "native" and st is not None and hip.dist_group is None and hip.fuse_optimiser
+                  and hip.rng == "philox" and hip.prof_events is None and self.bounds_method == "ray"
+                  and getattr(self.engine, "mailbox", None) is not None)
+        if not native:
+            start, end = self._timing_start(st)
 
         K = self.frames.T_WC_batch.shape[0]
         if len(self.frames) > self.window_size and self.incremental:
@@ -322,6 +326,12 @@
             _, fidx, nidx = hip.idx_cache
         norm_batch = self.frames.normal_batch if self.do_normal else None
         sc = self._sample_cfg()
+        if native:
+            if isinstance(fidx, tuple):
+                done = self._step_native(fidx, nidx, norm_batch, sc)
+                if done is not None:
+                    return done
+            start, end = self._timing_start(st)
         s = self._sample_raw(self.frames.depth_batch, self.frames.T_WC_batch, norm_batch, fidx,
                              nidx if norm_batch is not None else None, sc, want_T=False, reuse=True)
         self.active_pixels = _LazyCut(s)
@@ -363,6 +373,33 @@
                 float(eng.reduce_buf[eng.reduce_floats:].max())
             hip.prev_step_ms = float(np.float32(step_time))
         losses = StepLosses(mailbox, self.grad_weight != 0, self.eik_weight != 0)
+        hip.step_count += 1
+        self.tot_step_time += (1 / self.frac_time_perception) * (clock_ms / 1000.0)
+        self.steps_since_frame += 1
+        return losses, step_time
+
+    def _step_native(self, fidx, nidx, norm_batch, sc):
+        hip, eng, fal = self._hip, self.engine, self.frames.frame_avg_losses
+        if not (fal.is_contiguous() and fal.dtype == torch.float32 and (fal.device == hip.device or self._pinned(fal))):
+            return None
+        g = self.optimiser.param_groups[0]
+        optim = dict(lr=g["lr"], weight_decay=g["weight_decay"], betas=g["betas"], eps=g["eps"], frame_avg_out=fal,
+                     frame_avg_index=fidx)
+        noise = {} if self.noise_std is None else dict(noise_std=self.noise_std, noise_seed=hip.seed, noise_offset=hip.noise_count + 1)
+        r = eng.train_step_sync(self.frames.depth_batch, self.frames.T_WC_batch, norm_batch, fidx,
+                                nidx if norm_batch is not None else fidx, sc, self._loss_cfg(), hip.seed, hip.draw_count + 1,
+                                optim, **noise)
+        if r is None:
+            return None
+        s, step_time = r
+        hip.draw_count += 1
+        if noise:
+            hip.noise_count += 1
+        self.active_pixels = _LazyCut(s)
+        clock_ms = step_time
+        if hip.virtual_step_ms is not None:
+            clock_ms = step_time = float(hip.virtual_step_ms)
+        losses = StepLosses(eng.mailbox, self.grad_weight != 0, self.eik_weight != 0)
         hip.step_count += 1
         self.tot_step_time += (1 / self.frac_time_perception) * (clock_ms / 1000.0)
         self.steps_since_frame += 1
@@ -551,6 +588,13 @@
     return torch.device(trainer.device).type == "cuda" and torch.cuda.is_available() and os.path.exists(_ffi.LIB_PATH)
 
 
+def _step_path_from_env():
+    v = os.environ.get("ISDF_STEP_PATH", "native")
+    if v not in ("native", "python"):
+        raise ValueError("ISDF_STEP_PATH must be 'native' or 'python' (got %r)" % (v,))
+    return v
+
+
 def graft(trainer, rng="philox", seed=1, dist_group=None, fix_normal_window=False, fwd_operand="fp16x2",
           fuse_optimiser=True, virtual_step_ms=None, engine_factory=None, overlap_allreduce=False, bwd_operand=None, spill_operand=None, migrate_frames=True):
     if isinstance(trainer, HotPath) and getattr(trainer, "_hip", None) is not None:
@@ -599,6 +643,7 @@
                                 fuse_optimiser=bool(fuse_optimiser), device=dev, draw_count=0, noise_count=0,
                                 step_count=0, idx_cache=None, timing_events=None, prof_events=None,
                                 inline_window=True,
+                                step_path=_step_path_from_env(),
                                 overlap_allreduce=bool(overlap_allreduce) and dist_group is not None, split_event=None,
                                 comm_stream=None,
                                 virtual_step_ms=None if virtual_step_ms is None else float(virtual_step_ms),
```

Result: no change. 3952 train-steps/s, median of 4 (-0.1%).
